# jby1993/SelfReconCode

Hardware: AMD Instinct MI355X
Metric: train.py-equivalent iterations/sec (540x540, 2048 rays/frame x 3 frames per GPU; coarse stage at Adam lr 0.0001) (higher is better)
Workload: dtype f32

## Files before the change

include/selfrecon_hip.h:

```cpp
#ifndef SELFRECON_HIP_H_
#define SELFRECON_HIP_H_
#include <stdint.h>

#ifdef __cplusplus
extern "C" {
#endif

#define SR_OK 0
#define SR_EINVAL (-1)
#define SR_ELAUNCH (-2)
#define SR_ENOSPC (-3)

int sr_abi_version(void);
const char* sr_build_arch(void);
const char* sr_build_digest(void);

int sr_minv3x3_fwd_f32(const float* ms, float* invs, uint8_t* checks, int64_t n, void* stream);
int sr_minv3x3_fwd_f64(const double* ms, double* invs, uint8_t* checks, int64_t n, void* stream);
int sr_minv3x3_bwd_f32(const float* grads, const float* invs, float* outs, int64_t n, void* stream);
int sr_minv3x3_bwd_f64(const double* grads, const double* invs, double* outs, int64_t n, void* stream);

typedef struct {
  int64_t size[5];
  int64_t stride[5];
} sr_tensor5;

int sr_gridsample3d_fwd_f32(const float* input, sr_tensor5 in_d, const float* grid, sr_tensor5 grid_d,
                            float* output, sr_tensor5 out_d, void* stream);
int sr_gridsample3d_fwd_f64(const double* input, sr_tensor5 in_d, const double* grid, sr_tensor5 grid_d,
                            double* output, sr_tensor5 out_d, void* stream);
int sr_gridsample3d_bwd_f32(const float* input, sr_tensor5 in_d, const float* grid, sr_tensor5 grid_d,
                            const float* grad_output, sr_tensor5 gout_d,
                            float* grad_input , sr_tensor5 gin_d, float* grad_grid, void* stream);
int sr_gridsample3d_bwd_f64(const double* input, sr_tensor5 in_d, const double* grid, sr_tensor5 grid_d,
                            const double* grad_output, sr_tensor5 gout_d,
                            double* grad_input , sr_tensor5 gin_d, double* grad_grid, void* stream);
int sr_gridsample3d_fwd_f16(const void* input, sr_tensor5 in_d, const void* grid, sr_tensor5 grid_d, void* output, sr_tensor5 out_d,
                            void* stream);
int sr_gridsample3d_bwd_f16(const void* input, sr_tensor5 in_d, const void* grid, sr_tensor5 grid_d, const void* grad_output,
                            sr_tensor5 gout_d, void* grad_input , sr_tensor5 gin_d, void* grad_grid, void* stream);
int sr_gridsample3d_dbwd_f16(const void* gO_input , sr_tensor5 goi_d, const void* gO_grid, sr_tensor5 gog_d,
                             const void* input, sr_tensor5 in_d, const void* grid, sr_tensor5 grid_d, const void* grad_output,
                             sr_tensor5 gout_d, void* grad_input , sr_tensor5 gin_d, void* grad_grid,
                             void* grad_grad_output, void* stream);
int sr_gridsample3d_dbwd_f32(const float* gO_input , sr_tensor5 goi_d, const float* gO_grid, sr_tensor5 gog_d,
                             const float* input, sr_tensor5 in_d, const float* grid, sr_tensor5 grid_d,
                             const float* grad_output, sr_tensor5 gout_d,
                             float* grad_input , sr_tensor5 gin_d, float* grad_grid, float* grad_grad_output,
                             void* stream);
int sr_gridsample3d_dbwd_f64(const double* gO_input , sr_tensor5 goi_d, const double* gO_grid, sr_tensor5 gog_d,
                             const double* input, sr_tensor5 in_d, const double* grid, sr_tensor5 grid_d,
                             const double* grad_output, sr_tensor5 gout_d,
                             double* grad_input , sr_tensor5 gin_d, double* grad_grid, double* grad_grad_output,
                             void* stream);


#define SR_ACT_NONE 0
#define SR_ACT_SOFTPLUS100 1
#define SR_ACT_RELU 2
#define SR_EPI_FWD 0
#define SR_EPI_BWD 1
typedef struct {
  const float* A; int64_t lda;
  const float* B; int64_t ldb;
  float* C; int64_t ldc;
  int32_t M, N, K;
  const float* bias;
  int32_t group, act, mode;
  float out_scale;
  const float* aux; int64_t ldaux;
  int32_t naux_fwd;
  int32_t nact_bwd;
  float aux_scale;
} sr_gemm_args;
int sr_mlp_gemm_nt(const sr_gemm_args* host_args, void* stream);
int sr_mlp_gemm_nt_tile(int32_t M, int32_t ncols, int32_t* bm_out, int32_t* bn_out);

#define SR_CHAIN_MAX_LAYERS 10
typedef struct {
  int32_t nlayers;
  int32_t nprob[SR_CHAIN_MAX_LAYERS];
  sr_gemm_args g[SR_CHAIN_MAX_LAYERS][2];
  const int32_t* m_dev; int32_t m_mul;
  int32_t m_cap;
} sr_chain_args;
int sr_mlp_chain(const sr_chain_args* host_args, void* stream);

typedef struct {
  const float* Z; int64_t ldz;
  const float* A; int64_t lda;
  float* dW; int64_t lddw;
  float* partial;
  int32_t R, N, K, splits, accumulate;
  float* db; float* db_partial; int32_t group;
} sr_gemm_tn_args;
int64_t sr_mlp_gemm_tn_workspace_floats(int32_t R, int32_t N, int64_t lddw, int32_t* host_splits_out);
int sr_mlp_gemm_tn(const sr_gemm_tn_args* host_args, void* stream);
#define SR_TN_GROUP_MAX 12
typedef struct {
  int32_t n;
  sr_gemm_tn_args p[SR_TN_GROUP_MAX];
} sr_gemm_tn_group_args;
int sr_mlp_gemm_tn_group(const sr_gemm_tn_group_args* host_args, void* stream);

int sr_pe_embed(const float* x, int64_t P, int32_t L, const float* band_weights, const float* extra, int64_t ldextra,
                int32_t E, const int64_t* extra_index , int32_t group, float* out, int64_t ldo, void* stream);
int sr_pe_embed_bwd(const float* x, int64_t P, int32_t L, const float* band_weights, int32_t group, const float* gA0,
                    int64_t ldg, float* xbar, void* stream);

typedef struct {
  const float* p; const float* tp; int64_t P;
  const float* A; const float* trans; int32_t nframes;
  const int64_t* batch_inds; int64_t points_per_frame;
  const float* vol; int32_t D, H, W;
  float bmin[3], bmax[3];
  float* y;
  float* jac;
} sr_lbs_args;
int sr_lbs_fwd(const sr_lbs_args* host_args, void* stream);
int64_t sr_lbs_bwd_workspace_floats(int64_t P, int32_t nframes);
int sr_lbs_bwd(const sr_lbs_args* host_args, const float* ybar, float* pbar, float* Abar, float* transbar, float* partials, void* stream);
int sr_lbs_jac_bwd(const sr_lbs_args* host_args, const float* ybar, const float* Jbar, float* pbar, float* Abar, float* transbar, float* partials,
                   void* stream);

int sr_lbs_chain_fwd(const float* poses, int32_t B, const float* host_Js, const int32_t* host_parents, const float* host_init_pose,
                     float* G, float* A, void* stream);
int sr_lbs_chain_bwd(const float* poses, int32_t B, const float* host_Js, const int32_t* host_parents, const float* host_init_pose,
                     const float* Abar, const float* Gbar, float* posebar, void* stream);

typedef struct {
  int64_t M; int32_t group;
  const float* sdf4; int64_t ld_sdf;
  const float* off4; int64_t ld_off;
  const float* y; const float* jlbs;
  const float* rays; const float* cam;
  const float* p; float* p_out;
  uint8_t* converged;
  float dthreshold, athreshold, w1, w2;
} sr_newton_args;
int sr_newton_update(const sr_newton_args* host_args, void* stream);

typedef struct {
  int64_t M;
  const float* sdf; int64_t ld_sdf;
  const float* y; const float* jlbs;
  const float* rays; const float* cam;
  uint8_t* converged;
  float* t_out; int64_t ld_t; float* s_out;
  const float* grad_f; const float* grad_off;
  const float* p; float* p_out;
  float dthreshold, athreshold, w1, w2;
} sr_newton2_args;
int sr_newton_prepare(const sr_newton2_args* host_args, void* stream);
int sr_newton_apply(const sr_newton2_args* host_args, void* stream);

typedef struct {
  int32_t P, times;
  const float* p0; const float* rays; const int64_t* batch_inds;
  const float* cam;
  int32_t L_sdf; const float* w_sdf; int32_t L_def; const float* w_def;
  const float* conds; int64_t ld_conds; int32_t E;
  const float* A; const float* trans; int32_t nframes;
  const float* vol; int32_t D, H, W; float bmin[3], bmax[3];
  float dthreshold, athreshold, w1, w2;
  int32_t* live;
  float* x[2]; float* v[2]; int32_t* frame[2]; int32_t* orig[2];
  float* unit;
  float* a0; int64_t ld_a0; float* a0d; int64_t ld_a0d;
  const float* sdf_out; int64_t ld_sdf; const float* def_out; int64_t ld_def;
  uint8_t* conv; float* t; float* s;
  const float* a0bar; int64_t ld_a0bar; const float* skipbar; int64_t ld_skipbar; int32_t n_skip;
  const float* a0dbar; int64_t ld_a0dbar;
  float* p_out; uint8_t* conv_out;
} sr_refine_args;
int sr_refine_init(const sr_refine_args* host_args, void* stream);
int sr_refine_embed(const sr_refine_args* host_args, int32_t phase, void* stream);
int sr_refine_mid(const sr_refine_args* host_args, int32_t phase, int32_t mode, void* stream);
int sr_refine_finish(const sr_refine_args* host_args, int32_t phase, void* stream);


int64_t sr_mc_workspace_bytes(int32_t nx, int32_t ny, int32_t nz);
int sr_mc_count(const float* sdf, int32_t nx, int32_t ny, int32_t nz, float iso, void* workspace, uint32_t* counts_dev, void* stream);
int sr_mc_emit(const float* sdf, int32_t nx, int32_t ny, int32_t nz, float iso, const void* workspace, float xstep, float ystep,
               float zstep, float xmin, float ymin, float zmin, float* verts, int64_t* faces, void* stream);

int sr_svd3x3(const float* A, int64_t n, float* U, float* S, float* V, void* stream);

int sr_rows_pad(const float* a, int64_t lda, int32_t na, const float* b, int64_t ldb, int32_t nb, int64_t rows, int32_t group, float* dst, int64_t ldd,
                int32_t width, void* stream);
int64_t sr_rows_frame_sum_workspace_floats(int64_t P, int32_t E, int32_t n);
int sr_rows_frame_sum(const float* X, int64_t ldx, int64_t P, int32_t E, const int64_t* index, int32_t n, float* partial, float* out, void* stream);

#define SR_PACK_MAX_LAYERS 16
typedef struct { const float* v; const float* g; float* W; float* WT; float* norms; int32_t N, K; int64_t ldw, ldwt; } sr_pack_layer;
typedef struct { int32_t nlayers; sr_pack_layer layer[SR_PACK_MAX_LAYERS]; } sr_pack_table;
typedef struct { const float* dW; int64_t lddw; const float* v; const float* g; const float* norms; float* gv; float* gg;
                 const float* db; float* gb;
                 int32_t N, K, accumulate, pad_; } sr_unpack_layer;
typedef struct { int32_t nlayers; sr_unpack_layer layer[SR_PACK_MAX_LAYERS]; } sr_unpack_table;
int sr_pack_weights(const sr_pack_table* host_table, void* stream);
int sr_unpack_grads(const sr_unpack_table* host_table, void* stream);

#define SR_ADAM_MAX_TENSORS 64
typedef struct { float* p; const float* g; float* m; float* v; int64_t numel; float lr, bias1, inv_sqrt_bias2, pad_; } sr_adam_tensor;
typedef struct { int32_t ntensors; float beta1, beta2, eps;
                 float one_minus_beta1, one_minus_beta2;
                 int32_t pad_[2]; sr_adam_tensor tensor[SR_ADAM_MAX_TENSORS]; } sr_adam_table;
int sr_adam_step(const sr_adam_table* host_table, void* stream);

int sr_stream_stamp(uint64_t* out, void* stream);
int sr_stream_flag_set(uint32_t* flag, uint32_t value, void* stream);
int sr_stream_flag_wait(const uint32_t* flag, uint32_t value, uint32_t* timed_out, int32_t timeout_ms, void* stream);

int sr_interp2x3d_fwd_f32(const float* in, int64_t BC, int32_t d, int32_t h, int32_t w, float balance, float* out, uint8_t* is_boundary, void* stream);
int sr_interp2x3d_fwd_f64(const double* in, int64_t BC, int32_t d, int32_t h, int32_t w, float balance, double* out, uint8_t* is_boundary, void* stream);
int sr_interp2x3d_bwd_f32(const float* grad_out, int64_t BC, int32_t d, int32_t h, int32_t w, float* grad_in, void* stream);
int sr_interp2x3d_bwd_f64(const double* grad_out, int64_t BC, int32_t d, int32_t h, int32_t w, double* grad_in, void* stream);
int sr_seg3d_candidates(const uint8_t* is_boundary, const uint8_t* done, int32_t D, int32_t H, int32_t W, int64_t* out_index, uint64_t* count_dev,
                        void* stream);

int64_t sr_points_silhouette_workspace_bytes(int64_t nimg, int64_t pts_per_img, int32_t H, int32_t W, float radius);
int sr_points_silhouette_fwd(const float* xy_ndc, const float* z, int64_t nimg, int64_t pts_per_img, int32_t H, int32_t W, float radius,
                             int32_t K, float* mask, void* workspace, void* stream);
int sr_points_silhouette_bwd(const float* xy_ndc, const float* z, int64_t nimg, int64_t pts_per_img, int32_t H, int32_t W, float radius,
                             const void* workspace, const float* gmask, float* gxy, void* stream);
int sr_rasterize_meshes(const float* xy_ndc, const float* z, const int64_t* faces, int64_t nimg, int64_t V, int64_t F, int32_t H, int32_t W,
                        void* zbuf_u64, int64_t* pix_to_face, float* bary, float* zout, void* stream);

int sr_vertex_adjacency(const int64_t* faces, int64_t V, int64_t F, int64_t* offsets, int32_t* cursor, int32_t* nbr, void* stream);
int sr_vertex_normals(const float* verts, int64_t N, int64_t V, const int64_t* offsets, const int32_t* nbr, float* normals, void* stream);
int sr_shade_phong(const float* verts, const float* normals, const int64_t* faces, int64_t N, int64_t V, int64_t F, int32_t H, int32_t W,
                   const int64_t* pix_to_face, const float* bary, const float* cam_pos, const float* light_loc, const float* host_phong,
                   float* rgba, void* stream);

#define SR_STEP_MAX_FRAMES 8
typedef struct { const float* R; const float* T; const float* f; const float* c; float W, H, one_minus_inv_w, one_minus_inv_h; } sr_camera;
int sr_step_reduce_blocks(int64_t rows);
int sr_step_param_blocks(int64_t rows);
int sr_cam_project_ndc_fwd(const float* ps, int64_t n, const sr_camera* cam, float* xy, float* z, void* stream);
int sr_cam_project_ndc_bwd(const float* ps, int64_t n, const sr_camera* cam, const float* gxy, const float* gz, float* gps, float* partial,
                           float* gparams, void* stream);
int sr_cam_view_rays_fwd(const float* pixels, int64_t n, const sr_camera* cam, float* rays, void* stream);
int sr_cam_view_rays_bwd(const float* pixels, int64_t n, const sr_camera* cam, const float* grays, float* partial, float* gparams, void* stream);

int sr_cardinal_rays_fwd(const float* J, const float* v, int64_t n, float* out, uint8_t* ok, void* stream);
int sr_cardinal_rays_bwd(const float* J, const float* v, int64_t n, const float* gout, float* gJ, float* gv, void* stream);
int sr_deformed_normals(const float* J, const float* onx, int64_t n, float* out, void* stream);

#define SR_STEP_LOSS_SLOTS (1 + 2 * SR_STEP_MAX_FRAMES)
typedef struct { const int64_t* b; const int64_t* r; const int64_t* c; int64_t P; int32_t N, H, W; } sr_ray_pixels;
int sr_color_loss_fwd(const sr_ray_pixels* px, const float* colors, const float* gt, float* partial, float* out, void* stream);
int sr_color_loss_bwd(const sr_ray_pixels* px, const float* colors, const float* gt, const float* saved, const float* gloss, float* gcolors,
                      void* stream);
int sr_normal_loss_fwd(const sr_ray_pixels* px, const float* nx_raw, const float* J, const float* gt_normals, const float* R, const float* rays,
                       int weighted, float* partial, float* out, void* stream);
int sr_normal_loss_bwd(const sr_ray_pixels* px, const float* nx_raw, const float* J, const float* gt_normals, const float* R, const float* rays,
                       int weighted, const float* saved, const float* gloss, float* gnx_raw, float* gJ, void* stream);
int sr_eikonal_loss_fwd(const float* g, int64_t n, float* partial, float* out, void* stream);
int sr_eikonal_loss_bwd(const float* g, int64_t n, const float* gloss, float* gg, void* stream);
int sr_def_regu_loss_fwd(const float* S, int64_t n, float c, float* partial, float* out, void* stream);
int sr_def_regu_loss_bwd(const float* U, const float* S, const float* V, int64_t n, float c, const float* gloss, float* gJ, void* stream);
int sr_svd3x3_bwd(const float* U, const float* V, const float* gS, int64_t n, float* gJ, void* stream);
int sr_mask_iou_loss_fwd(const float* masks, const float* gt, int N, int64_t hw, float* partial, float* out, void* stream);
int sr_mask_iou_loss_bwd(const float* masks, const float* gt, int N, int64_t hw, const float* saved, const float* gloss, float* gmasks, void* stream);

int sr_implicit_solve(const float* grad_f, const float* J, const float* v, const float* grad_l, int64_t n, float* cot_f, float* rhs_tail, float* temp,
                      uint8_t* ok, void* stream);

int sr_uv_rasterize(const float* vt, const int64_t* ft, int64_t Vt, int64_t F, int32_t R, int32_t* face, float* bary, void* stream);
int sr_face_visibility(const int64_t* pix_to_face, const int64_t* faces, int64_t N, int64_t V, int64_t F, const float* xy_pix, const uint8_t* mask,
                       int32_t H, int32_t W, uint8_t* visible, void* stream);
int sr_view_alpha(const float* verts, const float* normals, const float* cam_pos, int64_t N, int64_t V, float* alpha, void* stream);
int sr_texture_accumulate(int64_t T, const int32_t* tface, const float* tbary, const int64_t* faces, int64_t F, int64_t V, int32_t N,
                          const uint8_t* visible, const float* alpha, const float* xy_pix, const float* images, int32_t H, int32_t W,
                          const int32_t* fids, int32_t agg_num, float cosv0, float* slot_cos, float* slot_rgb, int32_t* slot_view, int32_t* count,
                          float* min_cos, int32_t* min_idx, void* stream);
int sr_texture_resolve(int64_t T, const int32_t* texel, int32_t agg_num, float cosv0, int32_t check_num, const float* slot_cos,
                       const float* slot_rgb, const int32_t* slot_view, int32_t* count, uint8_t* mask_final, int32_t* view_id, float* tex_median,
                       void* stream);
int64_t sr_texture_fill_workspace_bytes(int32_t R);
int sr_texture_fill(const float* tex_median, const uint8_t* mask_final, const uint8_t* tex_mask, int32_t R, int32_t dilate, float* texture,
                    void* workspace, void* stream);

#define SR_QUADRIC_CLAMPED 1
#define SR_QUADRIC_NO_PLANES 2
int sr_meshprep_cell_faces(const int64_t* faces, int64_t F, const int64_t* vertex_map, int64_t V, int64_t C, int64_t* slot, void* stream);
int sr_meshprep_cell_quadric(const float* verts, int64_t V, const int64_t* faces, int64_t F, const int64_t* face_slots, const int64_t* face_offsets,
                             const int64_t* order, const int64_t* offsets, const int64_t* cells, int64_t C, const float* lo, float cell, int64_t nx,
                             int64_t ny, double reg, float* out, int32_t* flags, float* shift, void* stream);
int sr_meshprep_face_flips(const float* verts, int64_t V, const int64_t* faces, int64_t F, const float* new_verts, int64_t Vn,
                           const int64_t* new_faces, const int64_t* source, int64_t Fn, int64_t* counts, void* stream);
int sr_meshprep_bounds(const float* verts, int64_t V, int32_t* box, void* stream);
int sr_meshprep_cell_keys(const float* verts, int64_t V, const float* lo, float cell, int64_t nx, int64_t ny, int64_t nz, int64_t* key, void* stream);
int sr_meshprep_cell_mean(const float* verts, int64_t V, const int64_t* order, const int64_t* offsets, int64_t C, float* out, void* stream);
int sr_meshprep_face_keys(const int64_t* faces, int64_t F, const int64_t* vertex_map, int64_t V, int64_t Vn, int64_t* out_faces, int64_t* key_hi,
                          int64_t* key_lo, void* stream);
int sr_meshprep_face_first(const int64_t* key_hi, const int64_t* key_lo, const int64_t* perm, int64_t F, uint8_t* keep, void* stream);
int sr_chart_classify(const float* verts, int64_t V, const int64_t* faces, int64_t F, int32_t* cls, void* stream);
int sr_chart_edge_keys(const int64_t* faces, int64_t F, int64_t V, const int32_t* cls, int64_t* key, void* stream);
int sr_chart_hook(const int64_t* sorted_key, const int64_t* perm, int64_t n, const int32_t* parent, int32_t* next, int64_t F, int32_t* changed,
                  void* stream);
int sr_chart_jump(const int32_t* parent, int64_t F, int32_t* next, int32_t* changed, void* stream);
int sr_chart_bbox(const float* verts, int64_t V, const int64_t* faces, int64_t F, const int32_t* cls, const int64_t* chart, int64_t C, int32_t* box,
                  float* bbox_min, float* extent, void* stream);
int sr_chart_uv(const float* verts, int64_t V, const int64_t* faces, int64_t F, const int32_t* cls, const int64_t* chart, int64_t C,
                const float* bbox_min, const int64_t* origin, double scale, int32_t padding, int32_t R, float* vt, void* stream);
int sr_uv_overlap_count(const float* vt, const int64_t* ft, int64_t Vt, int64_t F, int32_t R, double eps, int32_t* count, int64_t* total,
                        void* stream);

int sr_collapse_vertex_quadrics(const float* verts, int64_t V, const int64_t* faces, int64_t F, const int64_t* slots, const int64_t* offsets,
                                double* quadrics, void* stream);
int sr_collapse_edge_keys(const int64_t* faces, int64_t F, int64_t V, int64_t* key, void* stream);
int sr_collapse_edge_heads(const int64_t* unique_key, const int64_t* offsets, int64_t E, const int64_t* perm, const int64_t* faces, int64_t F, int64_t V,
                           int64_t* edges, int32_t* count, int64_t* opposite, int32_t* locked, int64_t* directed, void* stream);
int sr_collapse_candidates(const float* verts, int64_t V, const int64_t* faces, int64_t F, const double* quadrics, const int64_t* slots,
                           const int64_t* offsets, const int64_t* neighbours, const int64_t* neighbour_offsets, const int64_t* edges,
                           const int32_t* count, const int64_t* opposite, const int32_t* locked, int64_t E, double reg, double flip_cos,
                           float* positions, int64_t* key, void* stream);
int sr_collapse_min1(const int64_t* edges, const int64_t* key, int64_t E, int64_t V, int64_t* m1, void* stream);
int sr_collapse_min2(const int64_t* edges, int64_t E, int64_t V, const int64_t* m1, int64_t* m2, void* stream);
int sr_collapse_select(const int64_t* edges, const int64_t* key, int64_t E, int64_t V, const int64_t* m2, uint8_t* selected, int64_t* record,
                       void* stream);
int sr_collapse_apply_vertices(const int64_t* edges, const float* positions, const uint8_t* selected, int64_t E, float* verts, int64_t V,
                               double* quadrics, int64_t* target, void* stream);
int sr_collapse_apply_faces(const int64_t* faces, int64_t F, const int64_t* target, int64_t V, int64_t* out_faces, uint8_t* keep, void* stream);
int sr_collapse_map_jump(const int64_t* parent, int64_t V, int64_t* next, int32_t* changed, void* stream);

int sr_texture_mips(const void* texture, int32_t is_u8, const uint8_t* valid, int32_t R, float* mips, void* stream);
int sr_texture_face_lod(const float* xy_pix, const int64_t* faces, const float* vt, const int64_t* ft, int64_t N, int64_t V, int64_t F,
                        int64_t Vt, int32_t R, float bias, int32_t L, float* lod, void* stream);
int sr_shade_textured(const int64_t* pix_to_face, const float* bary, int64_t N, int64_t F, int32_t H, int32_t W, const int64_t* ft,
                      const float* vt, int64_t Vt, const float* mips, int32_t R, int32_t L, const float* lod, const float* host_background,
                      const float* host_hole, const float* bg_image, float* rgba, float* coverage, void* stream);

#define SR_LBSW_MAX_K 32
int sr_lbsw_knn_blend(const float* verts, const float* vert_ws, int64_t nv, int32_t nj, int32_t k, int32_t W, int32_t H, int32_t D,
                      const float* bmin, const float* bmax, int32_t align_corners, float* field, void* stream);
int sr_lbsw_smooth(const float* src, float* dst, int32_t nj, int32_t W, int32_t H, int32_t D, void* stream);

#define SR_SMPL_BATCH_TILE 8
int sr_smpl_shape(const float* v_template, const float* shapedirs, const float* beta, int32_t B, int32_t nbeta, int64_t nv, float* v_shaped,
                  void* stream);
int64_t sr_smpl_regress_workspace_floats(int32_t B, int64_t nv, int32_t nk);
int sr_smpl_regress(const float* x, const float* reg, int32_t B, int64_t nv, int32_t nk, float* partial, float* out, void* stream);
int sr_smpl_pose(const float* theta, float* Rs, const float* J, const int32_t* host_parents, int32_t B, float* feature, float* J_transformed,
                 float* A, void* stream);
int sr_smpl_skin(const float* rest, int64_t rest_batch_stride, const float* posedirs, const float* feature, const float* weights, const float* A,
                 int32_t B, int64_t nv, float* verts, void* stream);

int sr_smpl_regress_bwd(const float* g_out, const float* reg, int32_t B, int64_t nv, int32_t nk, int32_t accumulate, float* g_x, void* stream);
int64_t sr_smpl_shape_bwd_workspace_floats(int32_t B, int32_t nbeta, int64_t nv);
int sr_smpl_shape_bwd(const float* shapedirs, const float* g_vshaped, int32_t B, int32_t nbeta, int64_t nv, float* partial, float* g_beta,
                      void* stream);
int64_t sr_smpl_skin_bwd_workspace_floats(int32_t B, int64_t nv);
int sr_smpl_skin_bwd(const float* rest, int64_t rest_batch_stride, const float* posedirs, const float* feature, const float* weights,
                     const float* A, const float* gV, int32_t B, int64_t nv, float* partial, float* g_rest, float* gA, float* g_feature,
                     void* stream);
int sr_smpl_pose_bwd(const float* theta, const float* Rs, const float* J, const float* A, const int32_t* host_parents, int32_t B,
                     const float* gA, const float* gJ_transformed, const float* g_feature, const float* gRs, float* g_theta, float* gRs_out,
                     float* gJ, void* stream);

int sr_keypoint_energy(const float* joints, const float* trans, const float* kp, const float* joint_weights, const float* host_camera,
                       float sigma, int32_t T, int32_t K, float* energy, float* g_joints, float* g_trans, int32_t* behind, void* stream);

#define SR_EDT_EMPTY 1073741824
int sr_edt(const uint8_t* mask, int32_t F, int32_t H, int32_t W, int32_t* d2, void* stream);
int sr_contour_flags(const uint8_t* mask, int32_t F, int32_t H, int32_t W, uint8_t* flags, void* stream);
int sr_silhouette_energy(const float* points, const int32_t* d2, const int32_t* samples, const int32_t* counts, const float* host_camera,
                         float sigma, float margin, int32_t F, int32_t V, int32_t S, int32_t H, int32_t W, float* xy, uint8_t* valid,
                         float* vres, int32_t* match, float* sres, float* e_in, float* e_cov, int32_t* outside, float* g_points, void* stream);

#define SR_MESHREG_LAP 1
#define SR_MESHREG_EDGE 2
#define SR_MESHREG_NORMAL 4
int64_t sr_meshreg_workspace_bytes(int64_t V, int64_t P);
int sr_meshreg_fwd(const float* verts, int64_t V, const int32_t* nbr_row, const int32_t* nbr, int64_t E, const int32_t* pairs, int64_t P,
                   int32_t terms, float target_length, float* lap_q, float* edge_g, float* pair_g, void* workspace, float* out, void* stream);
int sr_meshreg_bwd(int64_t V, const int32_t* nbr_row, const int32_t* nbr, int64_t E, const int32_t* pair_row, const int32_t* pair_ent, int64_t P,
                   const float* lap_q, const float* edge_g, const float* pair_g, const float* g_lap, const float* g_edge, const float* g_nc,
                   float* grad, void* stream);

#define SR_FRAMES_MAX_BATCH 16
#define SR_FRAMES_MAX_PIXELS 1073741824
struct sr_frame_ids_s {
  int32_t id[SR_FRAMES_MAX_BATCH];
};
typedef struct sr_frame_ids_s sr_frame_ids;
int sr_frames_fetch(const uint8_t* img_u8, const uint8_t* normal_u8, const uint8_t* mask_u8, int64_t pitch3, int64_t pitch1, int32_t F, int32_t H,
                    int32_t W, const sr_frame_ids* ids_by_value, const int64_t* ids_device, int32_t N, float* out_img, float* out_normal,
                    float* out_mask, void* stream);

#define SR_LOG_MAX_SLOTS 32
#define SR_LOG_EMPTY 0
#define SR_LOG_F32 1
#define SR_LOG_I64 2
#define SR_LOG_IMM 3
struct sr_log_slots_s {
  const void* src[SR_LOG_MAX_SLOTS];
  float imm[SR_LOG_MAX_SLOTS];
  uint8_t kind[SR_LOG_MAX_SLOTS];
};
typedef struct sr_log_slots_s sr_log_slots;
int sr_log_row(const sr_log_slots* slots_by_value, int32_t n, float* ring, int32_t ring_rows, int32_t ld, int64_t row, void* stream);

#define SR_JPEG_BLOCK_BYTES 208
int sr_jpeg_transform(const uint8_t* rgb, int32_t B, int32_t H, int32_t W, const uint16_t* qtab, int16_t* coef, void* stream);
int sr_jpeg_entropy(const int16_t* coef, int32_t B, int32_t H, int32_t W, const uint32_t* huff, uint32_t* bits, int64_t bits_dwords,
                    uint8_t* rowbuf, int64_t rowbuf_bytes, uint32_t* row_len, void* stream);
int sr_jpeg_gather(const uint8_t* rowbuf, const uint32_t* row_len, int32_t B, int32_t H, int32_t W, int64_t* row_start, uint8_t* out,
                   int64_t out_bytes, int64_t* offsets, void* stream);

int sr_surfdist_face_cells(const float* tri, int64_t F, const float* lo, float cell, int32_t nx, int32_t ny, int32_t nz, int64_t* count, void* stream);
int sr_surfdist_emit_pairs(const float* tri, int64_t F, const float* lo, float cell, int32_t nx, int32_t ny, int32_t nz, const int64_t* offset,
                           int64_t pairs, int64_t* key, int32_t* pair_face, void* stream);
int sr_surfdist_query(const float* points, int64_t P, const float* tri, int64_t F, const float* lo, float cell, int32_t nx, int32_t ny, int32_t nz,
                      const int64_t* cell_start, const int32_t* cell_faces, int64_t pairs, float* dist, int64_t* face, float* closest, void* stream);
int sr_surfdist_brute(const float* points, int64_t P, const float* tri, int64_t F, float* dist, int64_t* face, float* closest, void* stream);
int sr_mesh_sample(const float* tri, const double* cum_area, int64_t F, int64_t n, int64_t seed, float* points, int64_t* face, float* normals,
                   void* stream);

#define SR_ICP_MAX_BLOCKS 1024
#define SR_ICP_COLS 40
#define SR_ICP_HISTORY 6
#define SR_ICP_STATE 16
#define SR_ICP_DONE 12
int sr_icp_accumulate(const float* points, int64_t S, const float* tri, int64_t F, const float* lo, float cell, int32_t nx, int32_t ny, int32_t nz,
                      const int64_t* cell_start, const int32_t* cell_faces, int64_t pairs, const double* state, double ox, double oy, double oz,
                      double rho, float max_dist, int32_t measure, double* partial, int32_t blocks, void* stream);
int sr_icp_solve(const double* partial, int32_t blocks, double ox, double oy, double oz, double rho, int32_t scale, double tol, int32_t it,
                 int32_t iters, double* state, double* history, void* stream);
int sr_icp_score(const float* points, int64_t S, const double* table, int32_t N, const float* tri, int64_t F, const float* lo, float cell,
                 int32_t nx, int32_t ny, int32_t nz, const int64_t* cell_start, const int32_t* cell_faces, int64_t pairs, const float* trunc,
                 double* score, void* stream);

#ifdef __cplusplus
}
#endif
#endif
```

selfreconcode_amd/csrc/mlp_gemm.hip:

```cpp
#include "sr_common.h"
#include <stdlib.h>
#include <type_traits>

typedef float f32x16 __attribute__((ext_vector_type(16)));
typedef float f32x4 __attribute__((ext_vector_type(4)));
typedef int i32x4 __attribute__((ext_vector_type(4)));

__device__ __forceinline__ __amdgpu_buffer_rsrc_t sr_make_rsrc(const void* base, int64_t bytes) {
  return __builtin_amdgcn_make_buffer_rsrc(const_cast<void*>(base), 0, (int)(bytes < 0xFFFFFFFFll ? bytes : 0xFFFFFFFFll), 0x00020000);
}
__device__ __forceinline__ f32x4 sr_buffer_load16(__amdgpu_buffer_rsrc_t rsrc, uint32_t lane_off, uint32_t scalar_off) {
  return __builtin_bit_cast(f32x4, __builtin_amdgcn_raw_buffer_load_b128(rsrc, (int)lane_off, (int)scalar_off, 0));
}

namespace {

constexpr int BK = 32;
constexpr int LDSP = BK + 4;

__device__ __forceinline__ float fast_exp(float x) { return __builtin_amdgcn_exp2f(x * 1.4426950408889634f); }
__device__ __forceinline__ float fast_log(float x) { return __builtin_amdgcn_logf(x) * 0.6931471805599453f; }
__device__ __forceinline__ float softplus100(float z) {
  const float t = z * 100.0f;
  const float e = fast_exp(fminf(t, 20.0f));
  const float l = e < 1e-3f ? e * (1.0f - e * (0.5f - e * 0.33333334f)) : fast_log(1.0f + e);
  return t > 20.0f ? z : l * 0.01f;
}
__device__ __forceinline__ float dsoftplus100(float z) {
  const float t = z * 100.0f;
  const float e = fast_exp(fminf(t, 20.0f));
  return t > 20.0f ? 1.0f : e * __builtin_amdgcn_rcpf(e + 1.0f);
}
__device__ __forceinline__ void softplus100_from_stored(float x, float& d, float& c2) {
  const float em = fast_exp(-x);
  d = x < 1e-3f ? x * (1.0f - x * (0.5f - x * 0.16666667f)) : 1.0f - em;
  c2 = 100.0f * em;
}

template <int WM, int WN, int TM, int TN>
struct Cfg {
  static constexpr int kWaves = WM * WN;
  static constexpr int kThreads = kWaves * 64;
  static constexpr int BM = WM * TM * 32;
  static constexpr int BN = WN * TN * 32;
  static constexpr int kALoads = BM * (BK / 4) / kThreads;
  static constexpr int kBLoads = (BN * (BK / 4) + kThreads - 1) / kThreads;
  static constexpr int kOperandFloats = 2 * (BM + BN) * LDSP;
  static constexpr int kStageFloats = kWaves * TM * 32 * (TN * 32 + 4);
  static constexpr int kLdsFloats = kOperandFloats > kStageFloats ? kOperandFloats : kStageFloats;
};

template <int ROWS, int NLOADS, int THREADS>
struct TileLoader {
  const float* p[NLOADS];
  __amdgpu_buffer_rsrc_t rsrc;
  uint32_t off[NLOADS];
  int kq4;
  int K, kmax;
  __device__ __forceinline__ TileLoader(const float* __restrict__ P, int64_t ld, int R, int K_, int r0) : K(K_) {
    kq4 = (threadIdx.x & 7) * 4;
    kmax = ((K_ + 3) & ~3) - 4;
    const int rb = r0 < R ? r0 : R - 1;
    rsrc = sr_make_rsrc(P + (int64_t)rb * ld, (int64_t)(R - rb) * ld * 4);
#pragma unroll
    for (int j = 0; j < NLOADS; ++j) {
      int row = (threadIdx.x + j * THREADS) >> 3;
      if (row >= ROWS) row = ROWS - 1;
      int gr = r0 + row;
      if (gr >= R) gr = R - 1;
      p[j] = P + (int64_t)gr * ld;
      off[j] = (uint32_t)(((int64_t)(gr - rb) * ld + kq4) * 4);
    }
  }
  __device__ __forceinline__ void load(int k0, f32x4 (&reg)[NLOADS]) const {
    const int gk = k0 + kq4;
    const int gkc = gk < kmax ? gk : kmax;
#pragma unroll
    for (int j = 0; j < NLOADS; ++j) reg[j] = *reinterpret_cast<const f32x4*>(p[j] + gkc);
  }
  __device__ __forceinline__ void load_full(int k0, int klast, f32x4 (&reg)[NLOADS]) const {
    const uint32_t kc = (uint32_t)(k0 < klast ? k0 : klast) * 4u;
#pragma unroll
    for (int j = 0; j < NLOADS; ++j) reg[j] = sr_buffer_load16(rsrc, off[j], kc);
  }
  template <bool KTAIL = true>
  __device__ __forceinline__ void store(float* __restrict__ lds, int k0, const f32x4 (&reg)[NLOADS]) const {
    const int nvalid = K - (k0 + kq4);
#pragma unroll
    for (int j = 0; j < NLOADS; ++j) {
      const int idx = threadIdx.x + j * THREADS;
      const int row = idx >> 3;
      f32x4 v = reg[j];
      if (KTAIL) { v.x = nvalid > 0 ? v.x : 0.f; v.y = nvalid > 1 ? v.y : 0.f; v.z = nvalid > 2 ? v.z : 0.f; v.w = nvalid > 3 ? v.w : 0.f; }
      if (ROWS * 8 % THREADS == 0 || row < ROWS) *reinterpret_cast<f32x4*>(lds + row * LDSP + kq4) = v;
    }
  }
};

template <int WM, int WN, int TM, int TN, int G>
__device__ __forceinline__ void epilogue(const sr_gemm_args& g, f32x16 (&acc)[TM][TN], int m0, int n0, int wm, int wn,
                                         int li, int kh, float* __restrict__ stage) {
  constexpr int SP = TN * 32 + 4;
  const int ncols = g.N + g.naux_fwd;
  const float inv_aux_scale = 1.0f / g.aux_scale;
#pragma unroll
  for (int a = 0; a < TM; ++a) {
#pragma unroll
    for (int b = 0; b < TN; ++b) {
      const int col = n0 + (wn * TN + b) * 32 + li;
      if (col >= ncols) continue;
      const float bias = (g.bias && col < g.N) ? g.bias[col] : 0.f;
#pragma unroll
      for (int q = 0; q < 4; ++q) {
        const int r0 = m0 + (wm * TM + a) * 32 + 8 * q + 4 * kh;
        if (r0 >= g.M) continue;
        float v[4] = {acc[a][b][4 * q], acc[a][b][4 * q + 1], acc[a][b][4 * q + 2], acc[a][b][4 * q + 3]};
        float o[4];
        if (g.mode == SR_EPI_FWD) {
          if (col >= g.N) {
#pragma unroll
            for (int j = 0; j < 4; ++j) o[j] = (r0 + j < g.M) ? g.aux[(int64_t)(r0 + j) * g.ldaux + (col - g.N)] * g.out_scale : 0.f;
          } else {
#pragma unroll
            for (int s = 0; s < 4; s += G) {
              const float z = v[s] + bias;
              float d;
              if (g.act == SR_ACT_SOFTPLUS100) { o[s] = softplus100(z) * g.out_scale; d = (G > 1) ? dsoftplus100(z) : 0.f; }
              else if (g.act == SR_ACT_RELU) { o[s] = fmaxf(z, 0.f) * g.out_scale; d = z > 0.f ? 1.f : 0.f; }
              else { o[s] = z * g.out_scale; d = 1.f; }
#pragma unroll
              for (int tI = 1; tI < G; ++tI) o[s + tI] = d * v[s + tI] * g.out_scale;
            }
          }
        } else {
          if (col >= g.nact_bwd) {
#pragma unroll
            for (int j = 0; j < 4; ++j) o[j] = v[j] * g.out_scale;
          } else {
            float sv[4];
#pragma unroll
            for (int j = 0; j < 4; ++j) sv[j] = (r0 + j < g.M) ? g.aux[(int64_t)(r0 + j) * g.ldaux + col] : 0.f;
#pragma unroll
            for (int s = 0; s < 4; s += G) {
              float d, c2;
              if (g.act == SR_ACT_SOFTPLUS100) {
                softplus100_from_stored(100.0f * (sv[s] * inv_aux_scale), d, c2);
              } else if (g.act == SR_ACT_RELU) { d = sv[s] > 0.f ? 1.f : 0.f; c2 = 0.f; }
              else { d = 1.f; c2 = 0.f; }
              float cross = 0.f;
#pragma unroll
              for (int tI = 1; tI < G; ++tI) {
                cross += sv[s + tI] * v[s + tI];
                o[s + tI] = d * g.aux_scale * v[s + tI];
              }
              o[s] = d * g.aux_scale * v[s] + c2 * cross;
            }
          }
        }
        float* sp = stage + (a * 32 + 8 * q + 4 * kh) * SP + b * 32 + li;
#pragma unroll
        for (int j = 0; j < 4; ++j) sp[j * SP] = o[j];
      }
    }
  }
  __syncthreads();
  constexpr int QPR = TN * 8;
  constexpr int RPI = 64 / QPR;
  const int lane = kh * 32 + li;
  const int qc = lane % QPR, ro = lane / QPR;
  const int col0 = n0 + wn * TN * 32 + qc * 4;
#pragma unroll
  for (int i = 0; i < TM * 32 / RPI; ++i) {
    const int lr = i * RPI + ro;
    const int row = m0 + wm * TM * 32 + lr;
    if (row >= g.M || col0 >= ncols) continue;
    const f32x4 v = *reinterpret_cast<const f32x4*>(stage + lr * SP + qc * 4);
    float* dst = g.C + (int64_t)row * g.ldc + col0;
    if (col0 + 3 < ncols) {
      *reinterpret_cast<f32x4*>(dst) = v;
    } else {
      dst[0] = v.x;
      if (col0 + 1 < ncols) dst[1] = v.y;
      if (col0 + 2 < ncols) dst[2] = v.z;
    }
  }
}

template <int WM, int WN, int TM, int TN, int G, int MODE, int ACT>
__device__ __forceinline__ void epilogue_interior(const sr_gemm_args& g, f32x16 (&acc)[TM][TN], int m0, int n0, int wm, int wn, int li,
                                                  int kh, float* __restrict__ stage) {
  constexpr int SP = TN * 32 + 4;
  const float os = g.out_scale, as = g.aux_scale, inv_as = 1.0f / g.aux_scale;
#pragma unroll
  for (int a = 0; a < TM; ++a) {
#pragma unroll
    for (int b = 0; b < TN; ++b) {
      const int col = n0 + (wn * TN + b) * 32 + li;
      const float bias = (MODE == SR_EPI_FWD && g.bias) ? g.bias[col] : 0.f;
#pragma unroll
      for (int q = 0; q < 4; ++q) {
        const int r0 = m0 + (wm * TM + a) * 32 + 8 * q + 4 * kh;
        const float v[4] = {acc[a][b][4 * q], acc[a][b][4 * q + 1], acc[a][b][4 * q + 2], acc[a][b][4 * q + 3]};
        float o[4];
        if constexpr (MODE == SR_EPI_FWD) {
#pragma unroll
          for (int s = 0; s < 4; s += G) {
            const float z = v[s] + bias;
            float d = 1.f;
            if constexpr (ACT == SR_ACT_SOFTPLUS100) { o[s] = softplus100(z) * os; if (G > 1) d = dsoftplus100(z); }
            else if constexpr (ACT == SR_ACT_RELU) { o[s] = fmaxf(z, 0.f) * os; d = z > 0.f ? 1.f : 0.f; }
            else { o[s] = z * os; }
#pragma unroll
            for (int tI = 1; tI < G; ++tI) o[s + tI] = d * v[s + tI] * os;
          }
        } else {
          float sv[4];
          if constexpr (ACT != SR_ACT_NONE || G > 1) {
            const float* ap = g.aux + (int64_t)r0 * g.ldaux + col;
#pragma unroll
            for (int j = 0; j < 4; ++j) sv[j] = ap[(int64_t)j * g.ldaux];
          }
#pragma unroll
          for (int s = 0; s < 4; s += G) {
            float d = 1.f, c2 = 0.f;
            if constexpr (ACT == SR_ACT_SOFTPLUS100) softplus100_from_stored(100.0f * (sv[s] * inv_as), d, c2);
            else if constexpr (ACT == SR_ACT_RELU) d = sv[s] > 0.f ? 1.f : 0.f;
            float cross = 0.f;
#pragma unroll
            for (int tI = 1; tI < G; ++tI) {
              cross += sv[s + tI] * v[s + tI];
              o[s + tI] = d * as * v[s + tI];
            }
            o[s] = d * as * v[s] + c2 * cross;
          }
        }
        float* sp = stage + (a * 32 + 8 * q + 4 * kh) * SP + b * 32 + li;
#pragma unroll
        for (int j = 0; j < 4; ++j) sp[j * SP] = o[j];
      }
    }
  }
  __syncthreads();
  constexpr int QPR = TN * 8, RPI = 64 / QPR;
  const int lane = kh * 32 + li;
  const int qc = lane % QPR, ro = lane / QPR;
  float* dst = g.C + (int64_t)(m0 + wm * TM * 32 + ro) * g.ldc + n0 + wn * TN * 32 + qc * 4;
#pragma unroll
  for (int i = 0; i < TM * 32 / RPI; ++i)
    *reinterpret_cast<f32x4*>(dst + (int64_t)i * RPI * g.ldc) = *reinterpret_cast<const f32x4*>(stage + (i * RPI + ro) * SP + qc * 4);
}

template <int WM, int WN, int TM, int TN, int G, int MODE>
__device__ __forceinline__ void epilogue_interior_act(const sr_gemm_args& g, f32x16 (&acc)[TM][TN], int m0, int n0, int wm, int wn, int li,
                                                      int kh, float* __restrict__ stage) {
  if (g.act == SR_ACT_SOFTPLUS100) epilogue_interior<WM, WN, TM, TN, G, MODE, SR_ACT_SOFTPLUS100>(g, acc, m0, n0, wm, wn, li, kh, stage);
  else if (g.act == SR_ACT_RELU) epilogue_interior<WM, WN, TM, TN, G, MODE, SR_ACT_RELU>(g, acc, m0, n0, wm, wn, li, kh, stage);
  else epilogue_interior<WM, WN, TM, TN, G, MODE, SR_ACT_NONE>(g, acc, m0, n0, wm, wn, li, kh, stage);
}

struct NoProbe { __device__ __forceinline__ void operator()(int) const {} };
template <int WM, int WN, int TM, int TN, bool KTAIL = true, class Probe = NoProbe>
__device__ __forceinline__ void gemm_nt_tile(const sr_gemm_args& g, int wg, float* __restrict__ smem, Probe probe = Probe()) {
  using C_ = Cfg<WM, WN, TM, TN>;
  auto As = [&](int buf) -> float* { return smem + buf * (C_::BM * LDSP); };
  auto Bs = [&](int buf) -> float* { return smem + 2 * C_::BM * LDSP + buf * (C_::BN * LDSP); };

  const int tiles_n = (g.N + g.naux_fwd + C_::BN - 1) / C_::BN;
  const int tiles_m = (g.M + C_::BM - 1) / C_::BM;
  const int nwg = tiles_m * tiles_n;
  {
    const int q = nwg / 8, r = nwg % 8, xcd = wg % 8, loc = wg / 8;
    wg = (xcd < r ? xcd * (q + 1) : r * (q + 1) + (xcd - r) * q) + loc;
  }
  const int tn = wg % tiles_n, tm = wg / tiles_n;
  const int m0 = tm * C_::BM, n0 = tn * C_::BN;

  const int lane = threadIdx.x & 63, wave = threadIdx.x >> 6;
  const int wm = wave / WN, wn = wave % WN;
  const int li = lane & 31, kh = lane >> 5;

  f32x16 acc[TM][TN];
#pragma unroll
  for (int a = 0; a < TM; ++a)
#pragma unroll
    for (int b = 0; b < TN; ++b)
#pragma unroll
      for (int r = 0; r < 16; ++r) acc[a][b][r] = 0.f;

  const TileLoader<C_::BM, C_::kALoads, C_::kThreads> la(g.A, g.lda, g.M, g.K, m0);
  const TileLoader<C_::BN, C_::kBLoads, C_::kThreads> lb(g.B, g.ldb, g.N, g.K, n0);
  const int nk = (g.K + BK - 1) / BK;
  const int a_off = (wm * TM * 32 + li) * LDSP + kh * 4, b_off = (wn * TN * 32 + li) * LDSP + kh * 4;
  f32x4 fa0[2][TM], fb0[2][TN], fa1[2][TM], fb1[2][TN];
  auto read_frags = [&](const float* abuf, const float* bbuf, int kk0, f32x4 (&fa)[2][TM], f32x4 (&fb)[2][TN]) {
#pragma unroll
    for (int h = 0; h < 2; ++h) {
#pragma unroll
      for (int a = 0; a < TM; ++a) fa[h][a] = *reinterpret_cast<const f32x4*>(abuf + a_off + a * 32 * LDSP + (kk0 + h) * 8);
#pragma unroll
      for (int b = 0; b < TN; ++b) fb[h][b] = *reinterpret_cast<const f32x4*>(bbuf + b_off + b * 32 * LDSP + (kk0 + h) * 8);
    }
  };
  auto mfma_kk = [&](const f32x4 (&fa)[TM], const f32x4 (&fb)[TN]) {
#pragma unroll
    for (int e = 0; e < 4; ++e)
#pragma unroll
      for (int a = 0; a < TM; ++a)
#pragma unroll
        for (int b = 0; b < TN; ++b) acc[a][b] = __builtin_amdgcn_mfma_f32_32x32x2f32(fa[a][e], fb[b][e], acc[a][b], 0, 0, 0);
  };
  constexpr int kMem = C_::kALoads + C_::kBLoads;

  f32x4 ra0[C_::kALoads], rb0[C_::kBLoads], ra1[C_::kALoads], rb1[C_::kBLoads];
  const int klast = (nk - 1) * BK;
  auto load_tile = [&](int k0, f32x4 (&ar)[C_::kALoads], f32x4 (&br)[C_::kBLoads]) {
    if constexpr (KTAIL) { la.load(k0, ar); lb.load(k0, br); }
    else { la.load_full(k0, klast, ar); lb.load_full(k0, klast, br); }
  };
  load_tile(0, ra0, rb0);
  load_tile(BK, ra1, rb1);
  la.template store<KTAIL>(As(0), 0, ra0); lb.template store<KTAIL>(Bs(0), 0, rb0);
  __syncthreads();
  read_frags(As(0), Bs(0), 0, fa0, fb0);
  probe(0);
  auto step = [&](int t, f32x4 (&ain)[C_::kALoads], f32x4 (&bin)[C_::kBLoads], const f32x4 (&aout)[C_::kALoads],
                  const f32x4 (&bout)[C_::kBLoads]) {
    const int cur = t & 1;
    load_tile((t + 2) * BK, ain, bin);
    la.template store<KTAIL>(As(cur ^ 1), (t + 1) * BK, aout); lb.template store<KTAIL>(Bs(cur ^ 1), (t + 1) * BK, bout);
    read_frags(As(cur), Bs(cur), 2, fa1, fb1);
    mfma_kk(fa0[0], fb0[0]);
    mfma_kk(fa0[1], fb0[1]);
#pragma unroll
    for (int i = 0; i < kMem; ++i) {
      __builtin_amdgcn_sched_group_barrier(0x020, 1, 0);
      __builtin_amdgcn_sched_group_barrier(0x008, 1, 0);
    }
#pragma unroll
    for (int i = 0; i < kMem; ++i) {
      __builtin_amdgcn_sched_group_barrier(0x200, 1, 0);
      __builtin_amdgcn_sched_group_barrier(0x008, 1, 0);
    }
#pragma unroll
    for (int i = 0; i < 2 * (TM + TN); ++i) {
      __builtin_amdgcn_sched_group_barrier(0x100, 1, 0);
      __builtin_amdgcn_sched_group_barrier(0x008, 1, 0);
    }
    __builtin_amdgcn_sched_barrier(0);
    __syncthreads();
    read_frags(As(cur ^ 1), Bs(cur ^ 1), 0, fa0, fb0);
    __builtin_amdgcn_sched_barrier(0);
    mfma_kk(fa1[0], fb1[0]);
    mfma_kk(fa1[1], fb1[1]);
    __builtin_amdgcn_sched_barrier(0);
  };
  for (int t = 0; t < nk; t += 2) {
    step(t, ra0, rb0, ra1, rb1);
    if (t + 1 < nk) step(t + 1, ra1, rb1, ra0, rb0);
  }
  __syncthreads();
  probe(1);

  float* stage = smem + wave * (TM * 32 * (TN * 32 + 4));
  const bool interior = m0 + C_::BM <= g.M && n0 + C_::BN <= (g.mode == SR_EPI_FWD ? g.N : (g.nact_bwd < g.N ? g.nact_bwd : g.N));
  if (interior) {
    if (g.mode == SR_EPI_FWD) {
      switch (g.group) {
        case 1: epilogue_interior_act<WM, WN, TM, TN, 1, SR_EPI_FWD>(g, acc, m0, n0, wm, wn, li, kh, stage); break;
        case 2: epilogue_interior_act<WM, WN, TM, TN, 2, SR_EPI_FWD>(g, acc, m0, n0, wm, wn, li, kh, stage); break;
        default: epilogue_interior_act<WM, WN, TM, TN, 4, SR_EPI_FWD>(g, acc, m0, n0, wm, wn, li, kh, stage); break;
      }
    } else {
      switch (g.group) {
        case 1: epilogue_interior_act<WM, WN, TM, TN, 1, SR_EPI_BWD>(g, acc, m0, n0, wm, wn, li, kh, stage); break;
        case 2: epilogue_interior_act<WM, WN, TM, TN, 2, SR_EPI_BWD>(g, acc, m0, n0, wm, wn, li, kh, stage); break;
        default: epilogue_interior_act<WM, WN, TM, TN, 4, SR_EPI_BWD>(g, acc, m0, n0, wm, wn, li, kh, stage); break;
      }
    }
  } else {
    switch (g.group) {
      case 1: epilogue<WM, WN, TM, TN, 1>(g, acc, m0, n0, wm, wn, li, kh, stage); break;
      case 2: epilogue<WM, WN, TM, TN, 2>(g, acc, m0, n0, wm, wn, li, kh, stage); break;
      default: epilogue<WM, WN, TM, TN, 4>(g, acc, m0, n0, wm, wn, li, kh, stage); break;
    }
  }
  probe(2);
}

template <int WM, int WN, int TM, int TN, bool KTAIL>
__global__ __launch_bounds__(WM * WN * 64) __attribute__((amdgpu_waves_per_eu(2))) void gemm_nt_kernel(sr_gemm_args g) {
  extern __shared__ __attribute__((aligned(16))) float smem[];
  gemm_nt_tile<WM, WN, TM, TN, KTAIL>(g, blockIdx.x, smem);
}


using ChainCfg = Cfg<2, 2, 1, 1>;

constexpr int TBR = 32;
template <int ZW, int XW>
struct TnCfg {
  static constexpr int ZLD = ZW + 4, XLD = XW + 4;
  static constexpr int kZ = TBR * ZLD, kX = TBR * XLD;
  static constexpr int kLdsFloats = 2 * (kZ + kX);
  static constexpr int TLZ = TBR * (ZW / 4) / 256, TLX = TBR * (XW / 4) / 256;
  static constexpr int WN = XW / 64;
};

template <int ZW, int XW>
__device__ __forceinline__ void gemm_tn_body(const sr_gemm_tn_args& g, int rows_per_split, int bid, int nblocks, float* __restrict__ tn_smem) {
  using C = TnCfg<ZW, XW>;
  auto Zs = [&](int buf) -> float* { return tn_smem + buf * C::kZ; };
  auto Xs = [&](int buf) -> float* { return tn_smem + 2 * C::kZ + buf * C::kX; };
  const int tiles_k = (g.K + XW - 1) / XW;
  const int tiles_n = (g.N + ZW - 1) / ZW;
  int vb = bid;
  if ((nblocks & 7) == 0) vb = (bid & 7) * (nblocks >> 3) + (bid >> 3);
  const int tile = vb % (tiles_k * tiles_n), split = vb / (tiles_k * tiles_n);
  const int n0 = (tile / tiles_k) * ZW, k0 = (tile % tiles_k) * XW;
  const int r_begin = split * rows_per_split;
  const int r_end = min(g.R, r_begin + rows_per_split);
  const int lane = threadIdx.x & 63, wave = threadIdx.x >> 6;
  const int wm = wave / C::WN, wn = wave % C::WN, li = lane & 31, kh = lane >> 5;

  f32x16 acc[2][2];
#pragma unroll
  for (int a = 0; a < 2; ++a)
#pragma unroll
    for (int b = 0; b < 2; ++b)
#pragma unroll
      for (int r = 0; r < 16; ++r) acc[a][b][r] = 0.f;

  constexpr int TLZ = C::TLZ, TLX = C::TLX;
  constexpr int ZT = ZW / 4, XT = XW / 4;
  const int cqz = (threadIdx.x % ZT) * 4, lrz = threadIdx.x / ZT;
  const int cqx = (threadIdx.x % XT) * 4, lrx = threadIdx.x / XT;
  const int zmax = ((g.N + 3) & ~3) - 4, xmax = ((g.K + 3) & ~3) - 4;
  const float* zcol = g.Z + (n0 + cqz < zmax ? n0 + cqz : zmax);
  const float* xcol = g.A + (k0 + cqx < xmax ? k0 + cqx : xmax);
  f32x4 rz[TLZ], rx[TLX];
  const __amdgpu_buffer_rsrc_t zrsrc = sr_make_rsrc(g.Z + (int64_t)r_begin * g.ldz, (int64_t)(g.R - r_begin) * g.ldz * 4);
  const __amdgpu_buffer_rsrc_t xrsrc = sr_make_rsrc(g.A + (int64_t)r_begin * g.lda, (int64_t)(g.R - r_begin) * g.lda * 4);
  uint32_t zbyte[TLZ], xbyte[TLX];
#pragma unroll
  for (int j = 0; j < TLZ; ++j) zbyte[j] = (uint32_t)(((int64_t)(lrz + j * (256 / ZT)) * g.ldz + (zcol - g.Z)) * 4);
#pragma unroll
  for (int j = 0; j < TLX; ++j) xbyte[j] = (uint32_t)(((int64_t)(lrx + j * (256 / XT)) * g.lda + (xcol - g.A)) * 4);
  const int last_full = r_end - TBR;
  auto load = [&](int r0, auto tail) {
    if constexpr (decltype(tail)::value) {
#pragma unroll
      for (int j = 0; j < TLZ; ++j) {
        int gr = r0 + lrz + j * (256 / ZT);
        gr = gr < r_end ? gr : r_end - 1;
        rz[j] = *reinterpret_cast<const f32x4*>(zcol + (int64_t)gr * g.ldz);
      }
#pragma unroll
      for (int j = 0; j < TLX; ++j) {
        int gr = r0 + lrx + j * (256 / XT);
        gr = gr < r_end ? gr : r_end - 1;
        rx[j] = *reinterpret_cast<const f32x4*>(xcol + (int64_t)gr * g.lda);
      }
    } else {
      const int rc = r0 < last_full ? r0 : last_full;
      const uint32_t zo = (uint32_t)((int64_t)(rc - r_begin) * g.ldz * 4), xo = (uint32_t)((int64_t)(rc - r_begin) * g.lda * 4);
#pragma unroll
      for (int j = 0; j < TLZ; ++j) rz[j] = sr_buffer_load16(zrsrc, zbyte[j], zo);
#pragma unroll
      for (int j = 0; j < TLX; ++j) rx[j] = sr_buffer_load16(xrsrc, xbyte[j], xo);
    }
  };
  auto store = [&](int buf, int r0, auto tail) {
    float* zs = Zs(buf);
    float* xs = Xs(buf);
#pragma unroll
    for (int j = 0; j < TLZ; ++j) {
      const int row = lrz + j * (256 / ZT);
      f32x4 z = rz[j];
      if constexpr (decltype(tail)::value) {
        const bool ok = r0 + row < r_end;
        z.x = ok ? z.x : 0.f; z.y = ok ? z.y : 0.f; z.z = ok ? z.z : 0.f; z.w = ok ? z.w : 0.f;
      }
      *reinterpret_cast<f32x4*>(zs + row * C::ZLD + cqz) = z;
    }
#pragma unroll
    for (int j = 0; j < TLX; ++j) {
      const int row = lrx + j * (256 / XT);
      f32x4 x = rx[j];
      if constexpr (decltype(tail)::value) {
        const bool ok = r0 + row < r_end;
        x.x = ok ? x.x : 0.f; x.y = ok ? x.y : 0.f; x.z = ok ? x.z : 0.f; x.w = ok ? x.w : 0.f;
      }
      *reinterpret_cast<f32x4*>(xs + row * C::XLD + cqx) = x;
    }
  };

  constexpr int HS = TBR / 4;
  typedef float f32x2 __attribute__((ext_vector_type(2)));
  float z0a[HS], z1a[HS], x0a[HS], x1a[HS], z0b[HS], z1b[HS], x0b[HS], x1b[HS];
  const int zoff = kh * C::ZLD + wm * 64 + 2 * li, xoff = kh * C::XLD + wn * 64 + 2 * li;
  auto read_half = [&](int buf, int half, float (&z0)[HS], float (&z1)[HS], float (&x0)[HS], float (&x1)[HS]) {
    const float* zb = Zs(buf) + zoff + half * HS * 2 * C::ZLD;
    const float* xb = Xs(buf) + xoff + half * HS * 2 * C::XLD;
#pragma unroll
    for (int e = 0; e < HS; ++e) {
      const f32x2 z = *reinterpret_cast<const f32x2*>(zb + 2 * e * C::ZLD), x = *reinterpret_cast<const f32x2*>(xb + 2 * e * C::XLD);
      z0[e] = z.x; z1[e] = z.y; x0[e] = x.x; x1[e] = x.y;
    }
  };
  auto mfma_half = [&](const float (&z0)[HS], const float (&z1)[HS], const float (&x0)[HS], const float (&x1)[HS]) {
#pragma unroll
    for (int e = 0; e < HS; ++e) {
      acc[0][0] = __builtin_amdgcn_mfma_f32_32x32x2f32(z0[e], x0[e], acc[0][0], 0, 0, 0);
      acc[0][1] = __builtin_amdgcn_mfma_f32_32x32x2f32(z0[e], x1[e], acc[0][1], 0, 0, 0);
      acc[1][0] = __builtin_amdgcn_mfma_f32_32x32x2f32(z1[e], x0[e], acc[1][0], 0, 0, 0);
      acc[1][1] = __builtin_amdgcn_mfma_f32_32x32x2f32(z1[e], x1[e], acc[1][1], 0, 0, 0);
    }
  };

  const bool do_bias = g.db_partial != nullptr && k0 == 0;
  const float wodd = g.group == 4 ? 0.f : 1.f;
  float bsum0 = 0.f, bsum1 = 0.f;
  auto bias_half = [&](const float (&z0)[HS], const float (&z1)[HS]) {
#pragma unroll
    for (int e = 0; e < HS; ++e) {
      if (e & 1) { bsum0 += wodd * z0[e]; bsum1 += wodd * z1[e]; }
      else { bsum0 += z0[e]; bsum1 += z1[e]; }
    }
  };
  const int nsteps = (r_end - r_begin + TBR - 1) / TBR;
  auto run = [&](auto tail, auto bias) {
    load(r_begin, tail);
    store(0, r_begin, tail);
    load(r_begin + TBR, tail);
    __syncthreads();
    read_half(0, 0, z0a, z1a, x0a, x1a);
    for (int t = 0; t < nsteps; ++t) {
      const int cur = t & 1;
      store(cur ^ 1, r_begin + (t + 1) * TBR, tail);
      load(r_begin + (t + 2) * TBR, tail);
      read_half(cur, 1, z0b, z1b, x0b, x1b);
      mfma_half(z0a, z1a, x0a, x1a);
#pragma unroll
      for (int i = 0; i < TLZ + TLX; ++i) {
        __builtin_amdgcn_sched_group_barrier(0x200, 1, 0);
        __builtin_amdgcn_sched_group_barrier(0x008, 1, 0);
      }
#pragma unroll
      for (int i = 0; i < TLZ + TLX; ++i) {
        __builtin_amdgcn_sched_group_barrier(0x020, 1, 0);
        __builtin_amdgcn_sched_group_barrier(0x008, 1, 0);
      }
#pragma unroll
      for (int i = 0; i < HS; ++i) {
        __builtin_amdgcn_sched_group_barrier(0x100, 1, 0);
        __builtin_amdgcn_sched_group_barrier(0x008, 1, 0);
      }
      __builtin_amdgcn_sched_barrier(0);
      if constexpr (decltype(bias)::value) bias_half(z0a, z1a);
      __builtin_amdgcn_sched_barrier(0);
      __syncthreads();
      read_half(cur ^ 1, 0, z0a, z1a, x0a, x1a);
      __builtin_amdgcn_sched_barrier(0);
      mfma_half(z0b, z1b, x0b, x1b);
      if constexpr (decltype(bias)::value) bias_half(z0b, z1b);
      __builtin_amdgcn_sched_barrier(0);
    }
  };
  if (nsteps > 0) {
    const bool tail = ((r_end - r_begin) % TBR) != 0;
    if (tail) {
      if (do_bias) run(std::true_type{}, std::true_type{}); else run(std::true_type{}, std::false_type{});
    } else {
      if (do_bias) run(std::false_type{}, std::true_type{}); else run(std::false_type{}, std::false_type{});
    }
  }
  __syncthreads();
  if (do_bias) {
    float* red = Zs(0);
    if (wn == 0) {
      const bool use = kh == 0 || g.group == 1;
      red[kh * ZW + wm * 64 + 2 * li] = use ? bsum0 : 0.f;
      red[kh * ZW + wm * 64 + 2 * li + 1] = use ? bsum1 : 0.f;
    }
    __syncthreads();
    if (threadIdx.x < ZW && n0 + threadIdx.x < g.N) g.db_partial[(int64_t)split * g.N + n0 + threadIdx.x] = red[threadIdx.x] + red[threadIdx.x + ZW];
  }
  float* out = g.partial + (int64_t)split * g.N * g.lddw;
#pragma unroll
  for (int a = 0; a < 2; ++a)
#pragma unroll
    for (int b = 0; b < 2; ++b) {
      const int col = k0 + wn * 64 + 2 * li + b;
      if (col >= g.K) continue;
#pragma unroll
      for (int r = 0; r < 16; ++r) {
        const int row = n0 + wm * 64 + 2 * ((r & 3) + 8 * (r >> 2) + 4 * kh) + a;
        if (row < g.N) out[(int64_t)row * g.lddw + col] = acc[a][b][r];
      }
    }
}

template <int ZW, int XW>
__global__ __launch_bounds__(256) __attribute__((amdgpu_waves_per_eu(2))) void gemm_tn_kernel(sr_gemm_tn_args g, int rows_per_split) {
  extern __shared__ __attribute__((aligned(16))) float tn_smem[];
  gemm_tn_body<ZW, XW>(g, rows_per_split, blockIdx.x, gridDim.x, tn_smem);
}

struct TnGroup {
  int n;
  int first[SR_TN_GROUP_MAX + 1];
  int blocks[SR_TN_GROUP_MAX];
  int rows_per_split[SR_TN_GROUP_MAX];
  sr_gemm_tn_args p[SR_TN_GROUP_MAX];
};
__global__ __launch_bounds__(256) __attribute__((amdgpu_waves_per_eu(2))) void gemm_tn_group_kernel(TnGroup G) {
  extern __shared__ __attribute__((aligned(16))) float tn_smem[];
  int i = 0;
  while (i + 1 < G.n && (int)blockIdx.x >= G.first[i + 1]) ++i;
  const int bid = blockIdx.x - G.first[i];
  if (bid >= G.blocks[i]) return;
  gemm_tn_body<128, 128>(G.p[i], G.rows_per_split[i], bid, G.blocks[i], tn_smem);
}

static inline bool tn_narrow(int N, int64_t K) { return K <= 64 && N >= 256; }

__device__ __forceinline__ void slab_reduce_body(const float* __restrict__ partial, float* __restrict__ dW, int N,
                                                 int K, int64_t lddw, int splits, int accumulate,
                                                 const float* __restrict__ db_partial, float* __restrict__ db, int bid, int nblocks) {
  const int64_t total = (int64_t)N * lddw;
  const int64_t quads = total >> 2;
  const int64_t all = quads + (db ? N : 0);
  const f32x4* __restrict__ p4 = reinterpret_cast<const f32x4*>(partial);
  f32x4* __restrict__ d4 = reinterpret_cast<f32x4*>(dW);
  for (int64_t i = (int64_t)bid * blockDim.x + threadIdx.x; i < all; i += (int64_t)nblocks * blockDim.x) {
    if (i < quads) {
      const int col = (int)((i << 2) % lddw);
      f32x4 s = {0.f, 0.f, 0.f, 0.f};
      if (col < K) {
        const f32x4* src = p4 + i;
        int p = 0;
        for (; p + 8 <= splits; p += 8) {
          f32x4 v[8];
#pragma unroll
          for (int j = 0; j < 8; ++j) v[j] = src[(int64_t)(p + j) * quads];
#pragma unroll
          for (int j = 0; j < 8; ++j) s += v[j];
        }
        for (; p < splits; ++p) s += src[(int64_t)p * quads];
        if (col + 1 >= K) s.y = 0.f;
        if (col + 2 >= K) s.z = 0.f;
        if (col + 3 >= K) s.w = 0.f;
      }
      f32x4 o = {0.f, 0.f, 0.f, 0.f};
      if (accumulate) o = d4[i];
      d4[i] = o + s;
    } else {
      const int n = (int)(i - quads);
      float s = 0.f;
      for (int p = 0; p < splits; ++p) s += db_partial[(int64_t)p * N + n];
      db[n] = (accumulate ? db[n] : 0.f) + s;
    }
  }
}

__global__ __launch_bounds__(256) void slab_reduce_kernel(const float* __restrict__ partial, float* __restrict__ dW, int N,
                                                           int K, int64_t lddw, int splits, int accumulate,
                                                           const float* __restrict__ db_partial, float* __restrict__ db) {
  slab_reduce_body(partial, dW, N, K, lddw, splits, accumulate, db_partial, db, blockIdx.x, gridDim.x);
}

__global__ __launch_bounds__(256) void slab_reduce_group_kernel(TnGroup G) {
  int i = 0;
  while (i + 1 < G.n && (int)blockIdx.x >= G.first[i + 1]) ++i;
  const int bid = blockIdx.x - G.first[i];
  if (bid >= G.blocks[i]) return;
  const sr_gemm_tn_args& g = G.p[i];
  slab_reduce_body(g.partial, g.dW, g.N, g.K, g.lddw, g.R > 0 ? g.splits : 0, g.accumulate, g.db_partial, g.db, bid, G.blocks[i]);
}

}

static void nt_tile_choice(int M, int ncols, int* bm, int* bn) {
  auto cost = [&](int tm, int tn, double eff) {
    const int64_t wgs = sr_cdiv(M, tm) * sr_cdiv(ncols, tn);
    return (double)sr_cdiv(wgs, 256) * tm * tn / eff;
  };
  if (ncols <= 32) {
    const double c[3] = {cost(32, 32, 0.6), cost(64, 32, 0.8), cost(256, 32, 1.0)};
    *bn = 32;
    if (c[0] < c[1] && c[0] < c[2]) *bm = 32;
    else if (c[1] < c[2]) *bm = 64;
    else *bm = 256;
  } else {
    const double c[3] = {cost(64, 64, 0.92), cost(64, 128, 0.94), cost(128, 128, 1.0)};
    int pick = 1;
    for (int i = 1; i < 3; ++i) if (c[i] < c[pick - 1]) pick = i + 1;
    *bm = pick == 3 ? 128 : 64;
    *bn = pick == 1 ? 64 : 128;
  }
}

extern "C" {
int sr_mlp_gemm_nt(const sr_gemm_args* a, void* stream) {
  if (!a || a->M < 0 || a->N <= 0 || a->K <= 0) return SR_EINVAL;
  if (a->M == 0) return SR_OK;
  if (!a->A || !a->B || !a->C) return SR_EINVAL;
  if (a->group != 1 && a->group != 2 && a->group != 4) return SR_EINVAL;
  if ((a->lda & 3) || (a->ldb & 3) || (a->ldc & 3) || ((uintptr_t)a->A & 15) || ((uintptr_t)a->B & 15) || ((uintptr_t)a->C & 15)) return SR_EINVAL;
  if (a->mode != SR_EPI_FWD && a->mode != SR_EPI_BWD) return SR_EINVAL;
  if ((a->naux_fwd > 0 || a->mode == SR_EPI_BWD) && a->act != SR_ACT_NONE && !a->aux && a->mode == SR_EPI_BWD) return SR_EINVAL;
  if (a->mode == SR_EPI_FWD && a->naux_fwd > 0 && !a->aux) return SR_EINVAL;
  if (a->M == 0) return SR_OK;
  if (a->M % a->group) return SR_EINVAL;
  const int ncols = a->N + (a->mode == SR_EPI_FWD ? a->naux_fwd : 0);
  sr_gemm_args g = *a;
  if (g.mode != SR_EPI_FWD) g.naux_fwd = 0;
#define SR_NT_LAUNCH(WM, WN, TM, TN)                                                                                        \
  do {                                                                                                                      \
    using C_ = Cfg<WM, WN, TM, TN>;                                                                                         \
    const int nwg = (int)(sr_cdiv(g.M, C_::BM) * sr_cdiv(ncols, C_::BN));                                                   \
    if (g.K % BK)                                                                                                           \
      hipLaunchKernelGGL((gemm_nt_kernel<WM, WN, TM, TN, true>), dim3(nwg), dim3(C_::kThreads), C_::kLdsFloats * sizeof(float), \
                         (hipStream_t)stream, g);                                                                           \
    else                                                                                                                    \
      hipLaunchKernelGGL((gemm_nt_kernel<WM, WN, TM, TN, false>), dim3(nwg), dim3(C_::kThreads), C_::kLdsFloats * sizeof(float), \
                         (hipStream_t)stream, g);                                                                           \
  } while (0)
  int bm = 0, bn = 0;
  nt_tile_choice(g.M, ncols, &bm, &bn);
  switch (bm * 1024 + bn) {
    case 32 * 1024 + 32: SR_NT_LAUNCH(1, 1, 1, 1); break;
    case 64 * 1024 + 32: SR_NT_LAUNCH(2, 1, 1, 1); break;
    case 256 * 1024 + 32: SR_NT_LAUNCH(4, 1, 2, 1); break;
    case 64 * 1024 + 64: SR_NT_LAUNCH(2, 2, 1, 1); break;
    case 64 * 1024 + 128: SR_NT_LAUNCH(2, 2, 1, 2); break;
    default: SR_NT_LAUNCH(2, 2, 2, 2); break;
  }
#undef SR_NT_LAUNCH
  return sr_launch_status();
}

int sr_mlp_gemm_nt_tile(int32_t M, int32_t ncols, int32_t* bm, int32_t* bn) {
  if (M <= 0 || ncols <= 0 || !bm || !bn) return SR_EINVAL;
  nt_tile_choice(M, ncols, bm, bn);
  return SR_OK;
}

__global__ __launch_bounds__(ChainCfg::kThreads) __attribute__((amdgpu_waves_per_eu(2))) void mlp_layer_pair_kernel(sr_gemm_args g0, sr_gemm_args g1, int nprob,
                                                                                                                     const int32_t* __restrict__ m_dev, int m_mul) {
  extern __shared__ __attribute__((aligned(16))) float smem[];
  const int M = *m_dev * m_mul;
  if (M <= 0) return;
  const int rows = (M + ChainCfg::BM - 1) / ChainCfg::BM;
  const int t0 = rows * ((g0.N + (g0.mode == SR_EPI_FWD ? g0.naux_fwd : 0) + ChainCfg::BN - 1) / ChainCfg::BN);
  const int t1 = nprob > 1 ? rows * ((g1.N + (g1.mode == SR_EPI_FWD ? g1.naux_fwd : 0) + ChainCfg::BN - 1) / ChainCfg::BN) : 0;
  const int t = blockIdx.x;
  if (t >= t0 + t1) return;
  if (t < t0) { g0.M = M; if (g0.K % BK) gemm_nt_tile<2, 2, 1, 1, true>(g0, t, smem); else gemm_nt_tile<2, 2, 1, 1, false>(g0, t, smem); }
  else { g1.M = M; if (g1.K % BK) gemm_nt_tile<2, 2, 1, 1, true>(g1, t - t0, smem); else gemm_nt_tile<2, 2, 1, 1, false>(g1, t - t0, smem); }
}

int sr_mlp_chain(const sr_chain_args* a, void* stream) {
  if (!a || a->nlayers < 1 || a->nlayers > SR_CHAIN_MAX_LAYERS || !a->m_dev || a->m_mul < 1 || a->m_cap <= 0) return SR_EINVAL;
  for (int l = 0; l < a->nlayers; ++l) {
    if (a->nprob[l] < 1 || a->nprob[l] > 2) return SR_EINVAL;
    for (int p = 0; p < a->nprob[l]; ++p) {
      const sr_gemm_args& g = a->g[l][p];
      if (!g.A || !g.B || !g.C || g.N <= 0 || g.K <= 0 || g.group != a->m_mul) return SR_EINVAL;
      if ((g.lda & 3) || (g.ldb & 3) || (g.ldc & 3) || ((uintptr_t)g.A & 15) || ((uintptr_t)g.B & 15) || ((uintptr_t)g.C & 15)) return SR_EINVAL;
      if (g.mode != SR_EPI_FWD && g.mode != SR_EPI_BWD) return SR_EINVAL;
      if (g.mode == SR_EPI_BWD && g.naux_fwd != 0) return SR_EINVAL;
      if ((g.mode == SR_EPI_BWD && g.act != SR_ACT_NONE && !g.aux) || (g.mode == SR_EPI_FWD && g.naux_fwd > 0 && !g.aux)) return SR_EINVAL;
    }
  }
  const int64_t rows = sr_cdiv((int64_t)a->m_cap * a->m_mul, ChainCfg::BM);
  for (int l = 0; l < a->nlayers; ++l) {
    int64_t tiles = 0;
    for (int p = 0; p < a->nprob[l]; ++p) {
      const sr_gemm_args& g = a->g[l][p];
      tiles += rows * sr_cdiv(g.N + (g.mode == SR_EPI_FWD ? g.naux_fwd : 0), ChainCfg::BN);
    }
    hipLaunchKernelGGL(mlp_layer_pair_kernel, dim3((unsigned)tiles), dim3(ChainCfg::kThreads), ChainCfg::kLdsFloats * sizeof(float), (hipStream_t)stream,
                       a->g[l][0], a->g[l][a->nprob[l] > 1 ? 1 : 0], a->nprob[l], a->m_dev, a->m_mul);
  }
  return sr_launch_status();
}

int64_t sr_mlp_gemm_tn_workspace_floats(int32_t R, int32_t N, int64_t lddw, int32_t* splits_out) {
  const int tiles = tn_narrow(N, lddw) ? (int)sr_cdiv(N, 256) : (int)(sr_cdiv(N, 128) * sr_cdiv(lddw, 128));
  const int target = 512;
  int splits = (int)sr_cdiv(target, tiles);
  const int max_splits = (int)sr_cdiv(R, 384);
  if (splits > max_splits) splits = max_splits;
  if (splits < 1) splits = 1;
  if (splits_out) *splits_out = splits;
  return (int64_t)splits * N * lddw;
}

int sr_mlp_gemm_tn(const sr_gemm_tn_args* a, void* stream) {
  if (!a || !a->dW || !a->partial || a->R < 0 || a->N <= 0 || a->K <= 0 || a->splits < 1) return SR_EINVAL;
  if (a->R > 0 && (!a->Z || !a->A)) return SR_EINVAL;
  if ((a->ldz & 3) || (a->lda & 3) || ((uintptr_t)a->Z & 15) || ((uintptr_t)a->A & 15) || a->lddw < a->K) return SR_EINVAL;
  if ((a->lddw & 3) || ((uintptr_t)a->dW & 15) || ((uintptr_t)a->partial & 15)) return SR_EINVAL;
  if ((a->db != nullptr) != (a->db_partial != nullptr) || (a->db && a->group < 1)) return SR_EINVAL;
  const bool narrow = tn_narrow(a->N, a->lddw);
  const int tiles = narrow ? (int)sr_cdiv(a->N, 256) : (int)(sr_cdiv(a->N, 128) * sr_cdiv(a->K, 128));
  int rows_per_split = (int)sr_cdiv(a->R, a->splits);
  rows_per_split = (int)(sr_cdiv(rows_per_split, TBR) * TBR);
  if (a->R > 0) {
    using Narrow = TnCfg<256, 64>;
    using Square = TnCfg<128, 128>;
    if (narrow)
      hipLaunchKernelGGL((gemm_tn_kernel<256, 64>), dim3(tiles * a->splits), dim3(256), Narrow::kLdsFloats * sizeof(float), (hipStream_t)stream, *a,
                         rows_per_split);
    else
      hipLaunchKernelGGL((gemm_tn_kernel<128, 128>), dim3(tiles * a->splits), dim3(256), Square::kLdsFloats * sizeof(float), (hipStream_t)stream, *a,
                         rows_per_split);
  }
  const int64_t total = (int64_t)a->N * a->lddw / 4 + (a->db ? a->N : 0);
  sr_launch_stream(slab_reduce_kernel, total, 256, stream, a->partial, a->dW, a->N, a->K, a->lddw, a->R > 0 ? a->splits : 0, a->accumulate, a->db_partial,
                   a->db);
  return sr_launch_status();
}

static int tn_check(const sr_gemm_tn_args* a) {
  if (!a || !a->dW || !a->partial || a->R < 0 || a->N <= 0 || a->K <= 0 || a->splits < 1) return SR_EINVAL;
  if (a->R > 0 && (!a->Z || !a->A)) return SR_EINVAL;
  if ((a->ldz & 3) || (a->lda & 3) || ((uintptr_t)a->Z & 15) || ((uintptr_t)a->A & 15) || a->lddw < a->K) return SR_EINVAL;
  if ((a->lddw & 3) || ((uintptr_t)a->dW & 15) || ((uintptr_t)a->partial & 15)) return SR_EINVAL;
  if ((a->db != nullptr) != (a->db_partial != nullptr) || (a->db && a->group < 1)) return SR_EINVAL;
  return SR_OK;
}

int sr_mlp_gemm_tn_group(const sr_gemm_tn_group_args* a, void* stream) {
  if (!a || a->n < 1 || a->n > SR_TN_GROUP_MAX) return SR_EINVAL;
  TnGroup G, Rd;
  G.n = Rd.n = a->n;
  int nb = 0, nr = 0;
  bool any_rows = false;
  for (int i = 0; i < a->n; ++i) {
    const sr_gemm_tn_args& p = a->p[i];
    const int rc = tn_check(&p);
    if (rc != SR_OK) return rc;
    if (tn_narrow(p.N, p.lddw)) return SR_EINVAL;
    const int tiles = (int)(sr_cdiv(p.N, 128) * sr_cdiv(p.K, 128));
    int rows_per_split = (int)sr_cdiv(p.R, p.splits);
    rows_per_split = (int)(sr_cdiv(rows_per_split, TBR) * TBR);
    G.p[i] = Rd.p[i] = p;
    G.rows_per_split[i] = Rd.rows_per_split[i] = rows_per_split;
    G.first[i] = nb; G.blocks[i] = p.R > 0 ? tiles * p.splits : 0;
    nb += (int)(sr_cdiv(G.blocks[i], 8) * 8);
    const int64_t total = (int64_t)p.N * p.lddw / 4 + (p.db ? p.N : 0);
    Rd.first[i] = nr; Rd.blocks[i] = sr_stream_grid(total, 256);
    nr += Rd.blocks[i];
    any_rows = any_rows || p.R > 0;
  }
  G.first[a->n] = nb; Rd.first[a->n] = nr;
  using Square = TnCfg<128, 128>;
  if (any_rows && nb > 0)
    hipLaunchKernelGGL(gemm_tn_group_kernel, dim3(nb), dim3(256), Square::kLdsFloats * sizeof(float), (hipStream_t)stream, G);
  hipLaunchKernelGGL(slab_reduce_group_kernel, dim3(nr), dim3(256), 0, (hipStream_t)stream, Rd);
  return sr_launch_status();
}
}

namespace {
__global__ __launch_bounds__(256) void pe_embed_kernel(const float* __restrict__ x, int64_t P, int L, const float* __restrict__ w,
                                                        const float* __restrict__ extra, int64_t ldextra, int E,
                                                        const int64_t* __restrict__ extra_index, int group,
                                                        float* __restrict__ out, int64_t ldo) {
  const int width = 3 + 6 * L + E;
  const int64_t total = P * ldo;
  for (int64_t i = (int64_t)blockIdx.x * blockDim.x + threadIdx.x; i < total; i += (int64_t)gridDim.x * blockDim.x) {
    const int64_t p = i / ldo;
    const int c = (int)(i % ldo);
    float v = 0.f, t3[3] = {0.f, 0.f, 0.f};
    if (c < 3) {
      v = x[p * 3 + c];
      t3[c] = 1.f;
    } else if (c < 3 + 6 * L) {
      const int k = (c - 3) / 6, r = (c - 3) % 6, comp = r % 3;
      const float f = (float)(1 << k);
      const float a = x[p * 3 + comp] * f;
      const float wk = w[2 * k + (r >= 3)];
      if (r < 3) { v = wk * sinf(a); t3[comp] = wk * f * cosf(a); }
      else { v = wk * cosf(a); t3[comp] = -wk * f * sinf(a); }
    } else if (c < width) {
      const int64_t src = extra_index ? extra_index[p] : p;
      v = extra[src * ldextra + (c - 3 - 6 * L)];
    }
    out[(p * group) * ldo + c] = v;
    if (group == 4) {
      out[(p * 4 + 1) * ldo + c] = t3[0];
      out[(p * 4 + 2) * ldo + c] = t3[1];
      out[(p * 4 + 3) * ldo + c] = t3[2];
    }
  }
}
}

extern "C" int sr_pe_embed(const float* x, int64_t P, int32_t L, const float* band_weights, const float* extra, int64_t ldextra,
                           int32_t E, const int64_t* extra_index, int32_t group, float* out, int64_t ldo, void* stream) {
  if (P < 0 || L < 0 || L > 16 || E < 0 || (group != 1 && group != 4) || ldo < 3 + 6 * L + E) return SR_EINVAL;
  if (P == 0) return SR_OK;
  if (!x || !out || (L > 0 && !band_weights) || (E > 0 && !extra)) return SR_EINVAL;
  sr_launch_stream(pe_embed_kernel, P * ldo, 256, stream, x, P, L, band_weights, extra, ldextra, E, extra_index, group, out, ldo);
  return sr_launch_status();
}

namespace {
__global__ __launch_bounds__(256) void pe_embed_bwd_kernel(const float* __restrict__ x, int64_t P, int L, const float* __restrict__ w,
                                                            int group, const float* __restrict__ gA0, int64_t ldg, float* __restrict__ xbar) {
  for (int64_t i = (int64_t)blockIdx.x * blockDim.x + threadIdx.x; i < P * 3; i += (int64_t)gridDim.x * blockDim.x) {
    const int64_t p = i / 3;
    const int c = (int)(i % 3);
    const float xv = x[i];
    const float* g0 = gA0 + (p * group) * ldg;
    const float* gt = group == 4 ? gA0 + (p * 4 + 1 + c) * ldg : nullptr;
    float acc = g0[c];
    for (int k = 0; k < L; ++k) {
      const float f = (float)(1 << k);
      float sn, cs;
      sincosf(xv * f, &sn, &cs);
      const float ws = w[2 * k], wc = w[2 * k + 1];
      const int is = 3 + 6 * k + c, ic = is + 3;
      acc += f * (ws * cs * g0[is] - wc * sn * g0[ic]);
      if (gt) acc -= f * f * (ws * sn * gt[is] + wc * cs * gt[ic]);
    }
    xbar[i] = acc;
  }
}
}

extern "C" int sr_pe_embed_bwd(const float* x, int64_t P, int32_t L, const float* band_weights, int32_t group, const float* gA0,
                               int64_t ldg, float* xbar, void* stream) {
  if (P < 0 || L < 0 || L > 16 || (group != 1 && group != 4) || ldg < 3 + 6 * L) return SR_EINVAL;
  if (P == 0) return SR_OK;
  if (!x || !gA0 || !xbar || (L > 0 && !band_weights)) return SR_EINVAL;
  sr_launch_stream(pe_embed_bwd_kernel, P * 3, 256, stream, x, P, L, band_weights, group, gA0, ldg, xbar);
  return sr_launch_status();
}
```

selfreconcode_amd/mlp_engine.py:

```python
import collections
import contextlib
import ctypes
import math
import os
import weakref
import torch

from . import _lib

ACT_NONE, ACT_SOFTPLUS100, ACT_RELU = _lib.SR_ACT_NONE, _lib.SR_ACT_SOFTPLUS100, _lib.SR_ACT_RELU
EPI_FWD, EPI_BWD = _lib.SR_EPI_FWD, _lib.SR_EPI_BWD

TN_SIDE_STREAM = True
GROUP_TN_BELOW = 16384
DEBUG_TN_DELAY_MS = int(os.environ.get("SR_DEBUG_TN_DELAY_MS", "0"))
_TN_STREAMS = {}
_TN_PENDING = set()
_DELAY_FLAG = {}

DEFERRED_PARAM_GRADS = False

_PACK_CACHE = {}
_ENTRY_BY_PTR = {}

_INPUT_GRADS_ONLY = False


def pad4(n):
    return (n + 3) // 4 * 4


class LayerSpec:
    __slots__ = ("K", "N", "act", "out_scale", "nfill")

    def __init__(self, K, N, act, out_scale=1.0, nfill=0):
        self.K, self.N, self.act, self.out_scale, self.nfill = K, N, act, float(out_scale), nfill


class MLPSpec:

    def __init__(self, layers, K0):
        self.layers = layers
        self.K0 = K0

    @staticmethod
    def sdf(multires=6, width=512, nlin=9, skip_in=(4,), d_out=257):
        K0 = 3 + 6 * multires
        layers = []
        k = K0
        for l in range(nlin):
            last = l == nlin - 1
            n = d_out if last else width
            if (l + 1) in skip_in:
                layers.append(LayerSpec(k, n - K0, ACT_SOFTPLUS100, 1.0 / math.sqrt(2.0), nfill=K0))
            else:
                layers.append(LayerSpec(k, n, ACT_NONE if last else ACT_SOFTPLUS100))
            k = n
        return MLPSpec(layers, K0)

    @staticmethod
    def relu_mlp(K0, widths):
        layers, k = [], K0
        for i, n in enumerate(widths):
            layers.append(LayerSpec(k, n, ACT_NONE if i == len(widths) - 1 else ACT_RELU))
            k = n
        return MLPSpec(layers, K0)


_GemmRecord = collections.namedtuple("_GemmRecord", "e0 e1 flop rows overlap N K mode group")


class _GemmProfile:

    def __init__(self):
        self.overlap = False
        self.reset(enabled=False)

    def reset(self, enabled, reserve=0):
        self.enabled = enabled
        self.records, self.chains, self.pool = [], [], []
        for _ in range(reserve if enabled else 0):
            e0, e1 = torch.cuda.Event(enable_timing=True), torch.cuda.Event(enable_timing=True)
            e0.record(); e1.record()
            self.pool.append((e0, e1))

    def pair(self):
        return self.pool.pop() if self.pool else (torch.cuda.Event(enable_timing=True), torch.cuda.Event(enable_timing=True))

    def launch(self, name, args, stream, timed=True, what=None, marks=None):
        if not (timed and self.enabled):
            _lib.call(name, ctypes.byref(args), stream)
            return
        e0, e1 = self.pair()
        e0.record()
        _lib.call(name, ctypes.byref(args), stream)
        e1.record()
        if marks is not None:
            marks.append((e0, e1) + what)
        else:
            rows, N, K, mode, group = what
            self.records.append(_GemmRecord(e0, e1, 2.0 * rows * N * K, rows, self.overlap, N, K, mode, group))

    def summary(self):
        if not self.records:
            return {"tflops": 0.0, "launches": 0, "avg_us": 0.0, "avg_flop": 0.0}
        torch.cuda.synchronize()
        for marks, live, overlap in self.chains:
            lv = live.tolist()
            for e0, e1, phase, fpr in marks:
                self.records.append(_GemmRecord(e0, e1, fpr * lv[phase], lv[phase], overlap, 0, 0, "chain", 1))
        self.chains = []
        times = [r.e0.elapsed_time(r.e1) for r in self.records]

        def rate(sel):
            f = sum(r.flop for r, t, k in zip(self.records, times, sel) if k)
            ms = sum(t for t, k in zip(times, sel) if k)
            n = sum(1 for k in sel if k)
            return (f / (ms * 1e-3) / 1e12 if ms > 0 else 0.0), n, (ms * 1e3 / n if n else 0.0), (f / n if n else 0.0)

        nt = [r.mode != "tn" for r in self.records]
        alone = [k and not r.overlap for k, r in zip(nt, self.records)]
        tf, n, us, fl = rate(alone)
        tf_all, n_all, us_all, _ = rate(nt)
        tf_big, n_big, _, _ = rate([a and r.rows >= 65536 for a, r in zip(alone, self.records)])
        tf_tn, n_tn, us_tn, _ = rate([not k for k in nt])
        self._times = times
        f_nt = float(sum(r.flop for r, k in zip(self.records, nt) if k))
        f_tn = float(sum(r.flop for r, k in zip(self.records, nt) if not k))
        return {"tflops": round(tf, 3), "launches": n, "avg_us": round(us, 3), "avg_flop": round(fl, 1), "tflops_large": round(tf_big, 3),
                "launches_large": n_big, "tflops_all": round(tf_all, 3), "launches_all": n_all, "avg_us_all": round(us_all, 3),
                "avg_flop_all": round(f_nt / max(n_all, 1), 1), "flops_total": f_nt, "flops_total_tn": f_tn,
                "tflops_tn": round(tf_tn, 3), "launches_tn": n_tn, "avg_us_tn": round(us_tn, 3)}

    def by_shape(self):
        if not self.records:
            return []
        times = getattr(self, "_times", None) or [r.e0.elapsed_time(r.e1) for r in self.records]
        acc = {}
        for r, t in zip(self.records, times):
            a = acc.setdefault((r.rows, r.N, r.K, r.mode, r.group, bool(r.overlap)), [0, 0.0, 0.0])
            a[0] += 1; a[1] += r.flop; a[2] += t
        rows = [{"M": k[0], "N": k[1], "K": k[2], "mode": k[3], "group": k[4], "overlap": k[5], "launches": v[0], "flop": v[1], "ms": round(v[2], 4),
                 "tflops": round(v[1] / (v[2] * 1e-3) / 1e12, 2) if v[2] > 0 else 0.0} for k, v in acc.items()]
        rows.sort(key=lambda r: -r["ms"])
        return rows


PROFILE = _GemmProfile()


def set_gemm_args(a, A, B, C, M, N, K, bias, group, act, mode, out_scale=1.0, aux=None, naux_fwd=0, nact_bwd=0, aux_scale=1.0, pitches=None):
    lda, ldb, ldc, ldaux = pitches or (A.stride(0), B.stride(0), C.stride(0), 0 if aux is None else aux.stride(0))
    a.A, a.lda, a.B, a.ldb, a.C, a.ldc = A.data_ptr(), lda, B.data_ptr(), ldb, C.data_ptr(), ldc
    a.M, a.N, a.K = M, N, K
    a.bias = _lib.ptr(bias)
    a.group, a.act, a.mode, a.out_scale = group, act, mode, out_scale
    a.aux, a.ldaux, a.naux_fwd, a.nact_bwd, a.aux_scale = _lib.ptr(aux), ldaux, naux_fwd, nact_bwd, aux_scale


def _gemm_nt(A, lda, B, ldb, C, ldc, M, N, K, bias, group, act, mode, out_scale=1.0, aux=None, ldaux=0, naux_fwd=0,
             nact_bwd=0, aux_scale=1.0):
    a = _lib.SrGemmArgs()
    set_gemm_args(a, A, B, C, M, N, K, bias, group, act, mode, out_scale, aux, naux_fwd, nact_bwd, aux_scale, (lda, ldb, ldc, ldaux))
    PROFILE.launch("sr_mlp_gemm_nt", a, _lib.stream_of(C), M >= 128 and N > 32, (M, N, K, mode, group))


_TnProblem = collections.namedtuple("_TnProblem", "Z ldz A lda R N K lddw group dW db accumulate")


def _tn_workspace(R, N, lddw):
    splits = ctypes.c_int32(0)
    ws = _lib.raw("sr_mlp_gemm_tn_workspace_floats")(R, N, lddw, ctypes.byref(splits))
    return max(int(ws), 1), splits.value


def _set_tn_args(a, Z, ldz, A, lda, R, N, K, lddw, group, dW, db, accumulate, partial, ws, splits):
    a.Z, a.ldz, a.A, a.lda, a.dW, a.lddw, a.partial = Z.data_ptr(), ldz, A.data_ptr(), lda, dW.data_ptr(), lddw, partial
    a.R, a.N, a.K, a.splits, a.accumulate = R, N, K, splits, 1 if accumulate else 0
    a.db, a.db_partial, a.group = db.data_ptr(), partial + 4 * ws, group


def _gemm_tn(Z, ldz, A, lda, R, N, K, lddw, group=1, dW=None, db=None, accumulate=False):
    ws, splits = _tn_workspace(R, N, lddw)
    if dW is None:
        dW = torch.empty((N, lddw), dtype=torch.float32, device=Z.device)
    partial = torch.empty((ws + splits * N,), dtype=torch.float32, device=Z.device)
    if db is None:
        db = torch.empty((N,), dtype=torch.float32, device=Z.device)
    a = _lib.SrGemmTnArgs()
    _set_tn_args(a, Z, ldz, A, lda, R, N, K, lddw, group, dW, db, accumulate, partial.data_ptr(), ws, splits)
    PROFILE.launch("sr_mlp_gemm_tn", a, _lib.stream_of(Z), R >= 128 and N > 32, (R, N, K, "tn", group))
    return dW, db


def _tn_is_narrow(N, lddw):
    return lddw <= 64 and N >= 256


def _gemm_tn_group(problems):
    problems = [_TnProblem(*p) for p in problems]
    g = _lib.SrGemmTnGroupArgs()
    g.n = len(problems)
    sizes, total = [], 0
    for p in problems:
        ws, splits = _tn_workspace(p.R, p.N, p.lddw)
        sizes.append((ws, splits, total))
        total += (ws + splits * p.N + 3) // 4 * 4
    partial = torch.empty((total,), dtype=torch.float32, device=problems[0].Z.device)
    for a, p, (ws, splits, off) in zip(g.p, problems, sizes):
        _set_tn_args(a, *p, partial.data_ptr() + 4 * off, ws, splits)
    _lib.call("sr_mlp_gemm_tn_group", ctypes.byref(g), _lib.stream_of(partial))


def _debug_delay(device, ms):
    f = _DELAY_FLAG.get(str(device))
    if f is None:
        f = _DELAY_FLAG[str(device)] = torch.zeros(2, dtype=torch.int32, device=device)
    _lib.call('sr_stream_flag_wait', f.data_ptr(), 0x40000000, 0, ms, torch.cuda.current_stream(device).cuda_stream)


def _tn_stream(device):
    key = str(device)
    st = _TN_STREAMS.get(key)
    if st is None:
        st = _TN_STREAMS[key] = torch.cuda.Stream(device=device)
    return st


def _launch_on_tn_stream(device, problems):
    main, side = torch.cuda.current_stream(device), _tn_stream(device)
    ready = torch.cuda.Event()
    ready.record(main)
    side.wait_event(ready)
    with torch.cuda.stream(side):
        if DEBUG_TN_DELAY_MS:
            _debug_delay(device, DEBUG_TN_DELAY_MS)
        if len(problems) == 1:
            p = problems[0]
            _gemm_tn(*p[:9], dW=p.dW, db=p.db, accumulate=p.accumulate)
        else:
            _gemm_tn_group(problems)
    for p in problems:
        p.Z.record_stream(side); p.A.record_stream(side)
    _TN_PENDING.add(str(device))


def join_weight_gradient_stream():
    for key in list(_TN_PENDING):
        st = _TN_STREAMS[key]
        torch.cuda.current_stream(st.device).wait_stream(st)
    _TN_PENDING.clear()


def _check_mat(t, name):
    if t.dtype != torch.float32 or not t.is_cuda or t.dim() != 2 or t.stride(1) != 1 or (t.stride(0) % 4) or (t.data_ptr() % 16):
        raise RuntimeError(f"mlp_engine: {name} must be a GPU fp32 matrix with unit column stride, row pitch % 4 == 0 "
                           f"and 16-byte alignment (got {tuple(t.shape)}, strides {t.stride()}, {t.dtype}, {t.device})")


def _bias_segments(b0, R, group):
    if b0 is None or b0.dim() != 2:
        return None
    S = b0.shape[0]
    if S < 1 or R % S or (R // S) % group or b0.stride(1) != 1:
        raise RuntimeError(f"mlp_engine: segmented first-layer bias {tuple(b0.shape)} does not divide {R} rows of group {group}")
    return S, R // S


def forward(spec, A0, Ws, bs, group):
    _check_mat(A0, "A0")
    R = A0.shape[0]
    acts, X = [], A0
    seg = _bias_segments(bs[0], R, group)
    with _lib.on_device(A0.device):
        for l, L in enumerate(spec.layers):
            _check_mat(Ws[l], f"W{l}")
            C = torch.empty((R, pad4(L.N + L.nfill)), dtype=torch.float32, device=A0.device)
            if l == 0 and seg is not None:
                S, rs = seg
                for s in range(S):
                    Xs, Cs = X[s * rs:(s + 1) * rs], C[s * rs:(s + 1) * rs]
                    _gemm_nt(Xs, X.stride(0), Ws[l], Ws[l].stride(0), Cs, C.stride(0), rs, L.N, L.K, bs[0][s], group, L.act, EPI_FWD,
                             out_scale=L.out_scale, aux=A0[s * rs:(s + 1) * rs] if L.nfill else None, ldaux=A0.stride(0), naux_fwd=L.nfill)
            else:
                _gemm_nt(X, X.stride(0), Ws[l], Ws[l].stride(0), C, C.stride(0), R, L.N, L.K, bs[l], group, L.act, EPI_FWD,
                         out_scale=L.out_scale, aux=A0 if L.nfill else None, ldaux=A0.stride(0), naux_fwd=L.nfill)
            acts.append(C)
            X = C
    return acts


_DW_GROUPED, _DW_SIDE, _DW_SINK, _DW_SEGMENTED, _DW_AUTOGRAD = range(5)


def _weight_gradient_route(l, L, Ws, bs, seg, grouped):
    segmented = l == 0 and seg is not None
    sink = None
    if DEFERRED_PARAM_GRADS and Ws is not None:
        if not segmented:
            sink = _deferred_sink(Ws[l], bs[l])
        if sink is None and not Ws[l].requires_grad:
            e = _ENTRY_BY_PTR.get(Ws[l].data_ptr())
            if e is not None and any(r() is not None and r().requires_grad for r in e.src):
                raise RuntimeError("mlp_engine: a packed weight handed out without autograd node (deferred mode) met a layer call "
                                   "that has no deferred sink (bias that is not the layer's own leaf parameter?): its gradient would be lost")
    if sink is None:
        return (_DW_SEGMENTED if segmented else _DW_AUTOGRAD), None
    if grouped is not None and not _tn_is_narrow(L.N, pad4(L.K)) and len(grouped) < _lib.SR_TN_GROUP_MAX:
        return _DW_GROUPED, sink
    if TN_SIDE_STREAM and not PROFILE.enabled:
        return _DW_SIDE, sink
    return _DW_SINK, sink


def reverse(spec, A0, WTs, acts, Ybar, group, need_input_grad=True, need_param_grad=True, Ws=None, bs=None):
    _check_mat(Ybar, "Ybar")
    R = A0.shape[0]
    nl = len(spec.layers)
    dWs, dbs = [None] * nl, [None] * nl
    A0bar_extra = None
    Zbar = Ybar
    A0bar = None
    seg = _bias_segments(bs[0], R, group) if bs is not None else None
    grouped = [] if (0 < R < GROUP_TN_BELOW and TN_SIDE_STREAM and not PROFILE.enabled) else None
    with _lib.on_device(A0.device):
        for l in range(nl - 1, -1, -1):
            L = spec.layers[l]
            X = A0 if l == 0 else acts[l - 1]
            if need_param_grad:
                route, sink = _weight_gradient_route(l, L, Ws, bs, seg, grouped)
                if sink is not None:
                    p = _TnProblem(Zbar, Zbar.stride(0), X, X.stride(0), R, L.N, L.K, pad4(L.K), group, *sink)
                    if route == _DW_GROUPED:
                        grouped.append(p)
                    elif route == _DW_SIDE:
                        _launch_on_tn_stream(A0.device, [p])
                    else:
                        _gemm_tn(*p[:9], dW=p.dW, db=p.db, accumulate=p.accumulate)
                elif route == _DW_SEGMENTED:
                    S, rs = seg
                    dWs[0] = torch.empty((L.N, pad4(L.K)), dtype=torch.float32, device=A0.device)
                    dbs[0] = torch.zeros((S, L.N), dtype=torch.float32, device=A0.device)
                    for s in range(S):
                        _gemm_tn(Zbar[s * rs:(s + 1) * rs], Zbar.stride(0), X[s * rs:(s + 1) * rs], X.stride(0), rs, L.N, L.K, pad4(L.K), group,
                                 dW=dWs[0], db=dbs[0][s], accumulate=s > 0)
                else:
                    dWs[l], dbs[l] = _gemm_tn(Zbar, Zbar.stride(0), X, X.stride(0), R, L.N, L.K, pad4(L.K), group)
            if l > 0:
                Pv = spec.layers[l - 1]
                Znew = torch.empty((R, pad4(L.K)), dtype=torch.float32, device=A0.device)
                _gemm_nt(Zbar, Zbar.stride(0), WTs[l], WTs[l].stride(0), Znew, Znew.stride(0), R, L.K, L.N, None, group, Pv.act,
                         EPI_BWD, out_scale=Pv.out_scale, aux=acts[l - 1], ldaux=acts[l - 1].stride(0), nact_bwd=Pv.N,
                         aux_scale=Pv.out_scale)
                if Pv.nfill and need_input_grad:
                    A0bar_extra = Znew[:, Pv.N:Pv.N + Pv.nfill]
                Zbar = Znew
            elif need_input_grad:
                A0bar = torch.empty((R, pad4(L.K)), dtype=torch.float32, device=A0.device)
                _gemm_nt(Zbar, Zbar.stride(0), WTs[0], WTs[0].stride(0), A0bar, A0bar.stride(0), R, L.K, L.N, None, 1, ACT_NONE,
                         EPI_FWD)
                if A0bar_extra is not None:
                    A0bar[:, :A0bar_extra.shape[1]] += A0bar_extra
        if grouped:
            _launch_on_tn_stream(A0.device, grouped)
    return A0bar, dWs, dbs


def transpose_padded(W, K):
    N = W.shape[0]
    WT = torch.zeros((K, pad4(N)), dtype=W.dtype, device=W.device)
    WT[:, :N] = W[:, :K].t()
    return WT


def pad_cols(t, width):
    if t.shape[1] == width and t.is_contiguous():
        return t
    return torch.nn.functional.pad(t, (0, width - t.shape[1]))


def rows_pad(a, width, b=None, pair=False):
    ref = a if a is not None else b
    R = ref.shape[0]
    if not pair and a.shape[1] == width and a.stride(1) == 1 and a.stride(0) % 4 == 0 and a.data_ptr() % 16 == 0:
        return a
    srcs = []
    for t in (a, b):
        if t is not None and (t.stride(1) != 1 or t.dtype != torch.float32):
            t = t.contiguous().float()
        srcs.append(t)
    a, b = srcs
    out = torch.empty((R * (2 if pair else 1), width), dtype=torch.float32, device=ref.device)
    with _lib.on_device(ref.device):
        _lib.call("sr_rows_pad", _lib.ptr(a), 0 if a is None else a.stride(0), 0 if a is None else min(a.shape[1], width),
                  _lib.ptr(b), 0 if b is None else b.stride(0), 0 if b is None else min(b.shape[1], width),
                  R, 2 if pair else 1, _lib.ptr(out), width, width, _lib.stream_of(ref))
    return out


def rows_frame_sum(X, index, n):
    P, E = X.shape
    if X.dtype != torch.float32 or X.stride(1) != 1:
        X = X.float().contiguous()
    index = index.contiguous()
    out = torch.empty((n, E), dtype=torch.float32, device=X.device)
    part = _lib.workspace("sr_rows_frame_sum_workspace_floats", P, E, n, device=X.device, dtype=torch.float32)
    with _lib.on_device(X.device):
        _lib.call("sr_rows_frame_sum", _lib.ptr(X), X.stride(0), P, E, _lib.ptr(index), n, _lib.ptr(part), _lib.ptr(out), _lib.stream_of(X))
    return out


@contextlib.contextmanager
def input_grads_only():
    global _INPUT_GRADS_ONLY
    prev = _INPUT_GRADS_ONLY
    _INPUT_GRADS_ONLY = True
    try:
        yield
    finally:
        _INPUT_GRADS_ONLY = prev


class MLPCoreFunction(torch.autograd.Function):

    @staticmethod
    def forward(ctx, spec, A0, *wb):
        nl = len(spec.layers)
        Ws, bs = list(wb[:nl]), list(wb[nl:])
        acts = forward(spec, A0, Ws, bs, 1)
        ctx.spec = spec
        ctx.save_for_backward(A0, *wb, *acts[:-1])
        ctx.set_materialize_grads(False)
        NL = spec.layers[-1].N
        out = acts[-1]
        return out if out.shape[1] == NL else out[:, :NL]

    @staticmethod
    def backward(ctx, ybar):
        if ybar is None:
            return (None,) * (2 + 2 * len(ctx.spec.layers))
        saved = ctx.saved_tensors
        nl = len(ctx.spec.layers)
        A0, wb, acts = saved[0], saved[1:1 + 2 * nl], saved[1 + 2 * nl:]
        need_par = any(ctx.needs_input_grad[2:]) and not _INPUT_GRADS_ONLY
        outs = MLPCoreBackward.apply(ctx.spec, ctx.needs_input_grad[1], need_par, A0, ybar, *wb, *acts)
        return (None,) + tuple(outs)


class MLPCoreBackward(torch.autograd.Function):

    @staticmethod
    def forward(ctx, spec, need_in, need_par, A0, ybar, *rest):
        nl = len(spec.layers)
        Ws, bs, acts = list(rest[:nl]), list(rest[nl:2 * nl]), list(rest[2 * nl:])
        NL = spec.layers[-1].N
        yb = rows_pad(ybar, pad4(NL))
        WTs = [transposed_of(Ws[l], spec.layers[l].K) for l in range(nl)]
        A0bar, dWs, dbs = reverse(spec, A0, WTs, acts, yb, 1, need_in, need_par, Ws, bs)
        ctx.spec = spec
        ctx.save_for_backward(A0, ybar, *Ws, *bs)
        ctx.set_materialize_grads(False)
        if not need_par:
            dWs, dbs = [None] * nl, [None] * nl
        if A0bar is not None and A0bar.shape[1] != A0.shape[1]:
            A0bar = rows_pad(A0bar[:, :spec.K0], A0.shape[1])
        return (A0bar,) + tuple(dWs) + tuple(dbs)

    @staticmethod
    def backward(ctx, U, *param_cots):
        spec = ctx.spec
        nl = len(spec.layers)
        if any(c is not None for c in param_cots):
            raise NotImplementedError("selfreconcode_amd: differentiating MLP parameter gradients again is not supported "
                                      "(the reference only differentiates input gradients, network.py:102-114)")
        n_in = 5 + 2 * nl + (nl - 1)
        if U is None:
            return (None,) * n_in
        saved = ctx.saved_tensors
        A0, ybar = saved[0], saved[1]
        Ws, bs = list(saved[2:2 + nl]), list(saved[2 + nl:2 + 2 * nl])
        NL = spec.layers[-1].N
        R = A0.shape[0]
        A0i = rows_pad(A0, A0.shape[1], U, pair=True)
        acts2 = forward(spec, A0i, Ws, bs, 2)
        ydot = acts2[-1].view(R, 2, -1)[:, 1, :NL]
        ybi = rows_pad(None, pad4(NL), ybar, pair=True)
        WTs = [transposed_of(Ws[l], spec.layers[l].K) for l in range(nl)]
        need_in = ctx.needs_input_grad[3]
        need_par = any(ctx.needs_input_grad[5:5 + 2 * nl])
        A0bar2, dWs, dbs = reverse(spec, A0i, WTs, acts2, ybi, 2, need_in, need_par, Ws, bs)
        gA0 = A0bar2.view(R, 2, -1)[:, 0, :] if A0bar2 is not None else None
        if gA0 is not None and gA0.shape[1] != A0.shape[1]:
            gA0 = rows_pad(gA0[:, :spec.K0], A0.shape[1])
        return (None, None, None, gA0, ydot.contiguous()) + tuple(dWs) + tuple(dbs) + (None,) * (nl - 1)


def mlp_apply(spec, A0, Ws, bs):
    return MLPCoreFunction.apply(spec, A0, *Ws, *bs)


class _Pack:
    __slots__ = ("W", "WT", "norms", "sig", "src", "bias_param", "dW", "db", "bias", "fresh", "dirty")

    def __init__(self, W, WT, norms):
        self.W, self.WT, self.norms, self.sig, self.src = W, WT, norms, None, ()
        self.dW = self.db = self.bias = self.bias_param = None
        self.fresh, self.dirty = True, False


def _sig(*ts):
    return tuple((t.data_ptr(), t._version, tuple(t.shape)) for t in ts)


def _lin_params(lin):
    return (lin.weight_v, lin.weight_g) if hasattr(lin, "weight_g") else (lin.weight, None)


def _lin_sig(v, g):
    return _sig(v) if g is None else _sig(v, g)


def _raise_if_dirty(e):
    if e.dirty:
        raise RuntimeError("mlp_engine: parameters changed while deferred gradients were pending; call flush_param_grads() "
                           "before the optimizer step")


def _drop_entry(key):
    e = _PACK_CACHE.pop(key, None)
    if e is not None:
        _ENTRY_BY_PTR.pop(e.W.data_ptr(), None)


def _pack_entry(key, sig, build, owner=None):
    e = _PACK_CACHE.get(key)
    if e is None and owner is not None:
        weakref.finalize(owner, _drop_entry, key)
    if e is None or e.sig != sig:
        if e is not None:
            _raise_if_dirty(e)
            _drop_entry(key)
        e = build()
        e.sig = sig
        _PACK_CACHE[key] = e
        _ENTRY_BY_PTR[e.W.data_ptr()] = e
    return e


class PackWeightNorm(torch.autograd.Function):
    @staticmethod
    def forward(ctx, v, g):
        K = v.shape[1]

        def build():
            with torch.no_grad():
                w, norms = torch._weight_norm_interface(v, g, 0)
                W = pad_cols(w, pad4(K)).contiguous()
                return _Pack(W, transpose_padded(W, K), norms)
        e = _pack_entry(id(v), _sig(v, g), build, owner=v)
        e.src = (weakref.ref(v), weakref.ref(g))
        ctx.save_for_backward(v, g, e.norms)
        ctx.set_materialize_grads(False)
        return e.W.detach()

    @staticmethod
    def backward(ctx, gW):
        if gW is None:
            return None, None
        v, g, norms = ctx.saved_tensors
        gv, gg = torch.ops.aten._weight_norm_interface_backward(gW[:, :v.shape[1]].contiguous(), v, g, norms, 0)
        return gv, gg


class PackPlain(torch.autograd.Function):
    @staticmethod
    def forward(ctx, w):
        K = w.shape[1]

        def build():
            with torch.no_grad():
                W = pad_cols(w, pad4(K)).contiguous()
                if W.data_ptr() == w.data_ptr():
                    W = W.clone()
                return _Pack(W, transpose_padded(W, K), None)
        e = _pack_entry(id(w), _sig(w), build, owner=w)
        e.src = (weakref.ref(w),)
        ctx.K = K
        ctx.set_materialize_grads(False)
        return e.W.detach()

    @staticmethod
    def backward(ctx, gW):
        return None if gW is None else gW[:, :ctx.K]


def refresh_packs(lins):
    if not lins or not _lin_params(lins[0])[0].is_cuda:
        return
    stale = []
    for lin in lins:
        v, g = _lin_params(lin)
        e = _PACK_CACHE.get(id(v))
        if e is None:
            continue
        sig = _lin_sig(v, g)
        if e.sig != sig:
            _raise_if_dirty(e)
            if e.W.shape != (v.shape[0], pad4(v.shape[1])):
                continue
            stale.append((e, v, g, sig))
    for i in range(0, len(stale), _lib.SR_PACK_MAX_LAYERS):
        chunk = stale[i:i + _lib.SR_PACK_MAX_LAYERS]
        t = _lib.SrPackTable()
        t.nlayers = len(chunk)
        for j, (e, v, g, sig) in enumerate(chunk):
            L = t.layer[j]
            vv = v.detach()
            if not vv.is_contiguous():
                vv = vv.contiguous()
            L.v, L.g = _lib.ptr(vv), (0 if g is None else _lib.ptr(g.detach().contiguous()))
            L.W, L.WT, L.norms = _lib.ptr(e.W), _lib.ptr(e.WT), (0 if g is None else _lib.ptr(e.norms))
            L.N, L.K, L.ldw, L.ldwt = v.shape[0], v.shape[1], e.W.stride(0), e.WT.stride(0)
        with _lib.on_device(chunk[0][1].device), torch.no_grad():
            _lib.call("sr_pack_weights", ctypes.byref(t), _lib.stream_of(chunk[0][1]))
        for e, v, g, sig in chunk:
            e.sig = sig
        torch.autograd.graph.increment_version([t for e, _, _, _ in chunk for t in (e.W, e.WT, e.norms) if t is not None])


def pack_linear(lin):
    v, g = _lin_params(lin)
    if DEFERRED_PARAM_GRADS:
        e = _PACK_CACHE.get(id(v))
        b = lin.bias
        if e is not None and e.sig == _lin_sig(v, g) and e.src and b is not None and b.is_leaf and b.requires_grad:
            e.bias_param = b
            return e.W
    W = PackPlain.apply(v) if g is None else PackWeightNorm.apply(v, g)
    e = _ENTRY_BY_PTR.get(W.data_ptr())
    if e is not None:
        e.bias_param = lin.bias
    return W


def packed_weights_of(module, nlayers):
    d = module.__dict__
    mods = module._modules
    lins = [mods["lin" + str(l)] for l in range(nlayers)]
    params = []
    for lin in lins:
        P = lin._parameters
        v = P.get('weight_v')
        if v is not None:
            params.append(v); params.append(P['weight_g'])
        else:
            params.append(P['weight'])
        b = P.get('bias')
        if b is not None:
            params.append(b)
    key = (DEFERRED_PARAM_GRADS,) + tuple((id(p), p.data_ptr(), p._version, p.requires_grad) for p in params)
    hit = d.get('_sr_packs')
    if hit is not None and hit[0] == key:
        return list(hit[1]), list(hit[2])
    refresh_packs(lins)
    Ws, bs = [pack_linear(lin) for lin in lins], [lin.bias for lin in lins]
    if DEFERRED_PARAM_GRADS and all(W.grad_fn is None and not W.requires_grad and W.data_ptr() in _ENTRY_BY_PTR for W in Ws):
        d['_sr_packs'] = (key, list(Ws), list(bs))
    else:
        d.pop('_sr_packs', None)
    return Ws, bs


def transposed_of(W, K):
    e = _ENTRY_BY_PTR.get(W.data_ptr())
    if e is not None:
        WT = e.WT
        if WT.shape == (K, pad4(W.shape[0])):
            return WT
        if W.stride(0) == e.W.stride(0) and W.shape[0] <= e.W.shape[0] and K <= WT.shape[0] and pad4(W.shape[0]) <= WT.shape[1]:
            return WT[:K, :pad4(W.shape[0])]
    return transpose_padded(W, K)


def set_deferred_param_grads(flag):
    global DEFERRED_PARAM_GRADS
    flush_param_grads()
    DEFERRED_PARAM_GRADS = bool(flag)


def _deferred_sink(W, b):
    e = _ENTRY_BY_PTR.get(W.data_ptr())
    if e is None or b is None or not b.requires_grad or W.shape[0] > e.W.shape[0] or W.stride(0) != e.W.stride(0):
        return None
    n, full = W.shape[0], W.shape[0] == e.W.shape[0]
    if full:
        if not b.is_leaf:
            return None
    else:
        base = e.bias_param
        if base is None or not base.is_leaf or not base.requires_grad or b.data_ptr() != base.data_ptr():
            return None
        b = base
    if e.dW is None:
        e.dW = torch.empty_like(e.W)
        e.db = torch.empty((e.W.shape[0],), dtype=torch.float32, device=e.W.device)
        e.fresh = True
    if e.fresh and not full:
        e.dW.zero_(); e.db.zero_()
        e.fresh = False
    accumulate = not e.fresh
    e.fresh = False
    e.dirty = True
    e.bias = b
    return e.dW[:n], e.db[:n], accumulate


def flush_param_grads(only=None):
    todo = [e for e in _PACK_CACHE.values() if e.dirty and (only is None or id(e.src[0]()) in only)]
    if not todo:
        return
    join_weight_gradient_stream()
    for i in range(0, len(todo), _lib.SR_PACK_MAX_LAYERS):
        chunk = todo[i:i + _lib.SR_PACK_MAX_LAYERS]
        t = _lib.SrUnpackTable()
        t.nlayers = len(chunk)
        outs = []
        for j, e in enumerate(chunk):
            L = t.layer[j]
            src = tuple(r() for r in e.src)
            v = src[0]
            g = src[1] if len(src) == 2 else None
            acc = v.grad is not None and (g is None or g.grad is not None)
            gv = v.grad if acc else torch.empty_like(v, memory_format=torch.contiguous_format)
            gg = None
            if g is not None:
                gg = g.grad if acc else torch.empty_like(g, memory_format=torch.contiguous_format)
            if acc and (not gv.is_contiguous() or (gg is not None and not gg.is_contiguous())):
                acc = False
                gv = torch.empty_like(v, memory_format=torch.contiguous_format)
                gg = None if g is None else torch.empty_like(g, memory_format=torch.contiguous_format)
            vd = v.detach()
            if not vd.is_contiguous():
                vd = vd.contiguous()
            L.dW, L.lddw = _lib.ptr(e.dW), e.dW.stride(0)
            L.v, L.g, L.norms = _lib.ptr(vd), (0 if g is None else _lib.ptr(g.detach().contiguous())), (0 if g is None else _lib.ptr(e.norms))
            L.gv, L.gg, L.N, L.K, L.accumulate = _lib.ptr(gv), _lib.ptr(gg), v.shape[0], v.shape[1], 1 if acc else 0
            b = e.bias
            fold_bias = b.grad is not None and b.grad.is_contiguous() and b.grad.dtype == torch.float32
            L.db, L.gb = (_lib.ptr(e.db), _lib.ptr(b.grad)) if fold_bias else (0, 0)
            outs.append((e, v, g, gv, gg, acc, vd, fold_bias))
        dev = chunk[0].W.device
        with _lib.on_device(dev), torch.no_grad():
            _lib.call("sr_unpack_grads", ctypes.byref(t), torch.cuda.current_stream(dev).cuda_stream)
        for e, v, g, gv, gg, acc, _, fold_bias in outs:
            if not acc:
                v.grad = gv if v.grad is None else v.grad.add_(gv)
                if g is not None:
                    g.grad = gg if g.grad is None else g.grad.add_(gg)
            b = e.bias
            if fold_bias:
                torch.autograd.graph.increment_version(b.grad)
            elif b.grad is None:
                b.grad = e.db
                e.db = torch.empty_like(e.db)
            else:
                b.grad.add_(e.db)
            e.fresh = True
            e.dirty = False
```

selfreconcode_amd/model/Deformer.py:

```python
import ctypes
import os

import numpy as np
import torch
import torch.nn as nn
import torch.nn.functional as F

from .. import _lib
from .Embedder import embed_rows
from ..MCAcc.grid_sampler_mine import GridSamplerMine3dFunction
from ..mlp_engine import MLPSpec, mlp_apply, pad_cols, pad4, pack_linear
from ..utils.utils import resolve_band_weights


BATCH_FRAMES = True
HOIST_FRAME_CODE = True


_EYE3 = {}


def _eye3(device):
    e = _EYE3.get(device)
    if e is None:
        e = _EYE3[device] = torch.eye(3).to(device)
        if e.is_cuda:
            torch.cuda.current_stream(device).synchronize()
    return e


class CompositeDeformer(nn.Module):
    def __init__(self, deformers):
        super().__init__()
        self.N = len(deformers)
        self.defs = nn.ModuleList(deformers)

    def forward(self, ps, conds, batch_inds=None, **kwargs):
        assert self.N == len(conds)
        out = ps
        for cond, deformer in zip(conds, self.defs):
            out = deformer(out, cond, batch_inds, **kwargs)
        return out


class MLPTranslator(nn.Module):

    def __init__(self, feature_vector_size, multires, weight_norm=False):
        super().__init__()
        assert multires > 0
        dims = [3 + 6 * multires + feature_vector_size, 512, 512, 512, 512, 3]
        self.feature_vector_size = feature_vector_size
        self.multires = multires
        self.num_layers = len(dims)
        for l in range(0, self.num_layers - 1):
            lin = nn.Linear(dims[l], dims[l + 1])
            if weight_norm:
                print('MLPTranslator:weight norm can influence weight initialization, can not produce small weights as '
                      'initialization. Now do not use weight_norm')
            if l == self.num_layers - 2:
                torch.nn.init.normal_(lin.weight, mean=0., std=0.001)
                torch.nn.init.constant_(lin.bias, 0.)
            setattr(self, "lin" + str(l), lin)
        self.spec = MLPSpec.relu_mlp(dims[0], dims[1:])
        self.offset = None

    def packed_weights(self):
        from ..mlp_engine import packed_weights_of
        return packed_weights_of(self, len(self.spec.layers))

    def hoisted_first_layer(self, conds, frames=None):
        npe = 3 + 6 * self.multires
        W0 = self.lin0.weight
        Bf = conds.reshape(-1, self.feature_vector_size) @ W0[:, npe:].t() + self.lin0.bias
        if frames is not None and Bf.shape[0] != frames:
            raise ValueError(f"MLPTranslator: {Bf.shape[0]} condition codes for a batch of {frames} frames")
        W0p = pad_cols(W0[:, :npe], pad4(npe))
        spec = getattr(self, "_spec_pe", None)
        if spec is None:
            spec = self._spec_pe = MLPSpec.relu_mlp(npe, [L.N for L in self.spec.layers])
        return spec, W0p, Bf

    def forward(self, ps, conds, batch_inds=None, **kwargs):
        ratio = kwargs['ratio']['deformerRatio']
        ws = resolve_band_weights(self.multires, ratio)
        if batch_inds is None and HOIST_FRAME_CODE and ps.dim() == 3:
            spec, W0p, Bf = self.hoisted_first_layer(conds, ps.shape[0])
            Ws, bs = self.packed_weights()
            if BATCH_FRAMES:
                A0 = embed_rows(ps.reshape(-1, 3), self.multires, ws)
                self.offset = mlp_apply(spec, A0, [W0p] + Ws[1:], [Bf] + bs[1:]).view(ps.shape[0], ps.shape[1], 3)
                return ps[..., :3] + self.offset
            outs = []
            for p_f, B_f in zip(ps.unbind(0), Bf.unbind(0)):
                A0 = embed_rows(p_f, self.multires, ws)
                outs.append(mlp_apply(spec, A0, [W0p] + Ws[1:], [B_f] + bs[1:]))
            self.offset = torch.stack(outs, 0)
            return ps[..., :3] + self.offset
        if batch_inds is not None:
            flat, index, seg = ps, batch_inds, 0
        else:
            nb, nv = ps.shape[0], ps.shape[1]
            flat = ps.reshape(-1, 3)
            index = torch.arange(nb, device=ps.device).repeat_interleave(nv)
            seg = nv
        A0 = embed_rows(flat, self.multires, ws, extra=conds.reshape(-1, self.feature_vector_size), extra_index=index, segment=seg)
        Ws, bs = self.packed_weights()
        x = mlp_apply(self.spec, A0, Ws, bs)
        if batch_inds is not None:
            self.offset = x
            return ps[..., :3] + x
        self.offset = x.view(ps.shape[0], ps.shape[1], 3)
        return ps[..., :3] + self.offset


def getTranslatorNet(device, conf):
    return MLPTranslator(conf.get_int('condlen'), multires=conf.get_int('multires')).to(device)


def batch_rodrigues(theta):
    angle = torch.norm(theta + 1e-8, p=2, dim=1, keepdim=True)
    axis = theta / angle
    half = angle * 0.5
    q = torch.cat([torch.cos(half), torch.sin(half) * axis], dim=1)
    q = q / q.norm(p=2, dim=1, keepdim=True)
    w, x, y, z = q[:, 0], q[:, 1], q[:, 2], q[:, 3]
    w2, x2, y2, z2 = w * w, x * x, y * y, z * z
    wx, wy, wz, xy, xz, yz = w * x, w * y, w * z, x * y, x * z, y * z
    return torch.stack([w2 + x2 - y2 - z2, 2 * xy - 2 * wz, 2 * wy + 2 * xz,
                        2 * wz + 2 * xy, w2 - x2 + y2 - z2, 2 * yz - 2 * wx,
                        2 * xz - 2 * wy, 2 * wx + 2 * yz, w2 - x2 - y2 + z2], dim=1).view(-1, 3, 3)


def _tree_levels(parents):
    depth = [0] * len(parents)
    for i in range(1, len(parents)):
        depth[i] = depth[int(parents[i])] + 1
    return [[i for i in range(len(parents)) if depth[i] == d] for d in range(1, max(depth) + 1)]


class LBSkinner(nn.Module):

    def __init__(self, ws, bmins, bmaxs, Js, parents, init_pose=None, align_corners=False):
        super().__init__()

        def as_row(v):
            if isinstance(v, list):
                return torch.tensor(v, dtype=torch.float).view(1, 3)
            if isinstance(v, np.ndarray):
                return torch.from_numpy(v.astype(np.float32)).view(1, 3)
            return v.view(1, 3)
        self.register_buffer('b_min', as_row(bmins))
        self.register_buffer('b_max', as_row(bmaxs))
        ws = torch.from_numpy(ws.astype(np.float32)) if isinstance(ws, np.ndarray) else ws.to(torch.float)
        assert ws.dim() == 5 and ws.shape[0] == 1 and ws.shape[1] == 24
        self.register_buffer('ws', ws.contiguous(memory_format=torch.channels_last_3d))
        assert align_corners is False
        self.align_corners = align_corners
        self.register_buffer('Js', Js.view(24, 3).float())
        self.parents = [int(p) for p in parents]
        self._levels = _tree_levels(self.parents)
        if init_pose is None:
            raise NotImplementedError("the reference always builds the skinner with an init pose (network.py:843,851)")
        if isinstance(init_pose, np.ndarray):
            init_pose = torch.from_numpy(init_pose.astype(np.float32))
        if init_pose.numel() == 24 * 3:
            self.init_pose_inverse(batch_rodrigues(init_pose.view(-1, 3)).view(24, 3, 3), self.Js)
        else:
            self.register_buffer('init_pose', init_pose.view(24, 4, 4))

    def _apply(self, fn, *a, **k):
        out = super()._apply(fn, *a, **k)
        if not self.ws.is_contiguous(memory_format=torch.channels_last_3d):
            self.ws = self.ws.contiguous(memory_format=torch.channels_last_3d)
        return out

    def init_pose_inverse(self, init_pose, Js):
        R, T = [init_pose[0]], [Js[0]]
        for i in range(1, 24):
            pa = self.parents[i]
            R.append(R[pa] @ init_pose[i])
            T.append(R[pa] @ (Js[i] - Js[pa]) + T[pa])
        inv = torch.zeros(24, 4, 4)
        for i in range(24):
            inv[i, :3, :3] = R[i].t()
            inv[i, :3, 3] = -(R[i].t() @ T[i])
            inv[i, 3, 3] = 1.
        self.register_buffer('init_pose', inv)

    def _chain(self, poses):
        B = poses.shape[0]
        R = batch_rodrigues(poses.reshape(-1, 3)).view(B, 24, 3, 3)
        rel = self.Js.clone()
        rel[1:] = self.Js[1:] - self.Js[self.parents[1:]]
        local = torch.cat([torch.cat([R, rel.view(1, 24, 3, 1).expand(B, 24, 3, 1)], 3),
                           torch.cat([rel.new_zeros(3), rel.new_ones(1)]).view(1, 1, 1, 4).expand(B, 24, 1, 4)], 2)
        G = [None] * 24
        G[0] = local[:, 0]
        for level in self._levels:
            pa = torch.stack([G[self.parents[i]] for i in level], 1)
            prod = pa @ local[:, level]
            for n, i in enumerate(level):
                G[i] = prod[:, n]
        return torch.stack(G, 1)

    def _buffers_key(self):
        return tuple((t.data_ptr(), t._version) for t in (self.Js, self.init_pose, self.b_min, self.b_max))

    def _host_consts(self):
        key = self._buffers_key()
        if getattr(self, "_hc_key", None) != key:
            js = (ctypes.c_float * 72)(*self.Js.detach().cpu().view(-1).tolist())
            pa = (ctypes.c_int32 * 24)(*[max(p, 0) if i else 0 for i, p in enumerate(self.parents)])
            ip = (ctypes.c_float * 384)(*self.init_pose.detach().cpu().view(-1).tolist())
            self._hc = (js, pa, ip)
            self._box = (self.b_min.view(-1).tolist(), self.b_max.view(-1).tolist())
            self._hc_key = key
        return self._hc

    def _box_consts(self):
        self._host_consts()
        return self._box

    def posed_chain(self, poses):
        if poses.is_cuda:
            return _PosedChain.apply(self, poses)
        G = self._chain(poses)
        return G, G @ self.init_pose.view(1, 24, 4, 4)

    def posed_transforms(self, poses):
        return self.posed_chain(poses)[1]

    def posedSkeleton(self, conds):
        poses, trans = conds
        assert poses.shape[0] == trans.shape[0]
        return self.posed_chain(poses)[0][:, :, :3, 3]

    def fill_lbs_fields(self, a, A, trans):
        A12 = A[:, :, :3, :].contiguous()
        vol = self.ws.permute(0, 2, 3, 4, 1)
        assert vol.is_contiguous()
        a.A, a.trans, a.nframes = _lib.ptr(A12), _lib.ptr(trans), A.shape[0]
        a.vol, a.D, a.H, a.W = _lib.ptr(vol), vol.shape[1], vol.shape[2], vol.shape[3]
        box = self._box_consts()
        for i in range(3):
            a.bmin[i], a.bmax[i] = box[0][i], box[1][i]
        return A12, vol

    def _lbs_args(self, flat, A, trans, batch_inds, ppf, tp=None):
        a = _lib.SrLbsArgs()
        keep = self.fill_lbs_fields(a, A, trans)
        a.p, a.tp, a.P = _lib.ptr(flat), _lib.ptr(tp), flat.shape[0]
        a.batch_inds, a.points_per_frame = _lib.ptr(batch_inds), ppf
        return a, keep

    def fused(self, ps, A, trans, batch_inds=None, with_jac=False, tps=None):
        flat = ps.reshape(-1, 3).contiguous()
        P = flat.shape[0]
        tr = trans.contiguous()
        tp = None if tps is None else tps.reshape(-1, 3).contiguous()
        ppf = 0 if batch_inds is not None else (ps.shape[1] if ps.dim() == 3 else P)
        a, keep = self._lbs_args(flat, A, tr, batch_inds, ppf, tp)
        y = torch.empty_like(flat)
        jac = torch.empty((P, 3, 3), device=flat.device) if with_jac else None
        a.y, a.jac = _lib.ptr(y), _lib.ptr(jac)
        _lib.launch("sr_lbs_fwd", flat, ctypes.byref(a))
        return y.view(ps.shape), jac

    def forward(self, ps, conds, batch_inds=None, **kwargs):
        if type(ps) == list:
            tps, ps = ps
        else:
            tps = ps
        poses, trans = conds
        batch_size = poses.shape[0]
        assert batch_size == trans.shape[0]
        A = self.posed_transforms(poses)
        needs_graph = torch.is_grad_enabled() and (ps.requires_grad or tps.requires_grad or poses.requires_grad or trans.requires_grad)
        if not needs_graph:
            y, _ = self.fused(ps, A, trans, batch_inds, False, None if tps is ps else tps)
            return y
        if tps is ps:
            flat = ps.reshape(-1, 3)
            ppf = 0 if batch_inds is not None else ps.shape[1]
            y = _FusedLBS.apply(self, flat, A, trans, batch_inds, ppf)
            return y.view(ps.shape)
        return self._composite(ps, tps, A, trans, batch_inds)

    def _composite(self, ps, tps, A, trans, batch_inds):
        batch_size = A.shape[0]
        nps = 2. * (tps.reshape(-1, 3) - self.b_min) / (self.b_max - self.b_min) - 1.
        w = GridSamplerMine3dFunction.apply(self.ws, nps.reshape(1, 1, 1, -1, 3)).view(24, -1).transpose(0, 1)
        A12 = A[:, :, :3, :].reshape(batch_size, 24, 12)
        if batch_inds is None:
            nb, pnum, _ = ps.shape
            assert nb == batch_size
            T = torch.matmul(w.view(nb, pnum, 24), A12).view(nb, pnum, 3, 4)
            return (T[..., :3] @ ps.unsqueeze(-1)).squeeze(-1) + T[..., 3] + trans.view(-1, 1, 3)
        p = ps.reshape(-1, 3)
        Tall = (w @ A12.permute(1, 0, 2).reshape(24, batch_size * 12)).view(-1, batch_size, 12)
        T = torch.gather(Tall, 1, batch_inds.view(-1, 1, 1).expand(-1, 1, 12)).view(-1, 3, 4)
        return (T[..., :3] @ p.unsqueeze(-1)).squeeze(-1) + T[..., 3] + trans[batch_inds]

    def fused_backward(self, flat, A, batch_inds, ppf, ybar, need_p, need_A, need_t, Jbar=None):
        N, dev = A.shape[0], flat.device
        a, keep = self._lbs_args(flat, A, None, batch_inds, ppf)
        cots = [None if ybar is None else ybar.contiguous().float()] + ([] if Jbar is None else [Jbar.contiguous().float()])
        pbar = torch.empty_like(flat) if need_p else None
        Abar = torch.empty((N, 24, 12), device=dev) if need_A else None
        tbar = torch.empty((N, 3), device=dev) if (need_t and ybar is not None) else None
        part = _lib.workspace("sr_lbs_bwd_workspace_floats", flat.shape[0], N, device=dev, dtype=torch.float32)
        _lib.launch("sr_lbs_bwd" if Jbar is None else "sr_lbs_jac_bwd", flat, ctypes.byref(a), *cots, pbar, Abar, tbar, part)
        return pbar, Abar, tbar


def _frame_major(flat, A, batch_inds):
    return flat if batch_inds is not None else flat.view(A.shape[0], -1, 3)


def _cotangent_4x4(Abar):
    return None if Abar is None else F.pad(Abar.view(-1, 24, 3, 4), (0, 0, 0, 1))


class _PosedChain(torch.autograd.Function):
    @staticmethod
    def forward(ctx, skin, poses):
        p = poses.detach().contiguous().float().view(-1, 24, 3)
        B = p.shape[0]
        G = torch.empty((B, 24, 4, 4), dtype=torch.float32, device=p.device)
        A = torch.empty_like(G)
        js, pa, ip = skin._host_consts()
        _lib.launch("sr_lbs_chain_fwd", p, p, B, js, pa, ip, G, A)
        ctx.skin = skin
        ctx.save_for_backward(p)
        ctx.pshape = poses.shape
        ctx.set_materialize_grads(False)
        return G, A

    @staticmethod
    def backward(ctx, Gbar, Abar):
        if Gbar is None and Abar is None:
            return None, None
        (p,) = ctx.saved_tensors
        js, pa, ip = ctx.skin._host_consts()
        out = torch.empty_like(p)
        gb = None if Gbar is None else Gbar.contiguous().float()
        ab = None if Abar is None else Abar.contiguous().float()
        _lib.launch("sr_lbs_chain_bwd", p, p, p.shape[0], js, pa, ip, ab, gb, out)
        return None, out.view(ctx.pshape)


class _FusedLBS(torch.autograd.Function):

    @staticmethod
    def forward(ctx, skin, flat, A, trans, batch_inds, ppf):
        flat = flat.contiguous()
        y, _ = skin.fused(_frame_major(flat, A, batch_inds), A, trans, batch_inds, False, None)
        ctx.skin, ctx.ppf = skin, ppf
        ctx.save_for_backward(flat, A, trans, batch_inds)
        return y.reshape(-1, 3)

    @staticmethod
    def backward(ctx, ybar):
        flat, A, trans, batch_inds = ctx.saved_tensors
        skin = ctx.skin
        need_p, need_A, need_t = ctx.needs_input_grad[1], ctx.needs_input_grad[2], ctx.needs_input_grad[3]
        if torch.is_grad_enabled():
            ps = _frame_major(flat, A, batch_inds)
            y2 = skin._composite(ps, ps, A, trans, batch_inds).reshape(-1, 3)
            ins = [t for t, n in ((flat, need_p), (A, need_A), (trans, need_t)) if n]
            gs = list(torch.autograd.grad(y2, ins, ybar, create_graph=True, allow_unused=True))
            out = [gs.pop(0) if n else None for n in (need_p, need_A, need_t)]
            return None, out[0], out[1], out[2], None, None
        pbar, Abar, tbar = skin.fused_backward(flat, A, batch_inds, ctx.ppf, ybar, need_p, need_A, need_t)
        return None, pbar, _cotangent_4x4(Abar), tbar, None, None


class _LBSValueJacobian(torch.autograd.Function):

    @staticmethod
    def forward(ctx, skin, q, A, trans, batch_inds, ppf):
        flat = q.reshape(-1, 3).contiguous().float()
        y, J = skin.fused(_frame_major(flat, A, batch_inds), A, trans, batch_inds, True, None)
        ctx.skin, ctx.ppf = skin, ppf
        ctx.save_for_backward(flat, A, batch_inds)
        ctx.set_materialize_grads(False)
        return y.reshape(-1, 3), J

    @staticmethod
    def backward(ctx, ybar, Jbar):
        flat, A, batch_inds = ctx.saved_tensors
        skin = ctx.skin
        if ybar is None and Jbar is None:
            return (None,) * 6
        need_q, need_A, need_t = ctx.needs_input_grad[1], ctx.needs_input_grad[2], ctx.needs_input_grad[3]
        Jb = torch.zeros((flat.shape[0], 3, 3), device=flat.device) if Jbar is None else Jbar
        qbar, Abar, tbar = skin.fused_backward(flat, A, batch_inds, ctx.ppf, ybar, need_q, need_A, need_t, Jb)
        return None, qbar, _cotangent_4x4(Abar), tbar, None, None


def deformer_value_jacobian(deformer, ps, defconds, batch_inds, ratio):
    tr, skin = deformer.defs[0], deformer.defs[1]
    d_cond, (poses, trans) = defconds[0], defconds[1]
    q, Jq = translator_value_jacobian(tr, ps, d_cond, batch_inds, ratio)
    A = skin.posed_transforms(poses)
    y, Jl = _LBSValueJacobian.apply(skin, q, A, trans, batch_inds, 0)
    from ..utils.utils import small_matmul
    return y, small_matmul(Jl, Jq)


def is_fused_composite(deformer):
    return (isinstance(deformer, CompositeDeformer) and deformer.N == 2 and isinstance(deformer.defs[0], MLPTranslator)
            and isinstance(deformer.defs[1], LBSkinner))


class TranslatorValueJacobian(torch.autograd.Function):

    @staticmethod
    def forward(ctx, tr, ratio, x, conds, index, segment, spec, *wb):
        from .. import mlp_engine as me
        from .Embedder import band_weight_tensor
        spec = spec or tr.spec
        nl = len(spec.layers)
        Ws, bs = list(wb[:nl]), list(wb[nl:])
        flat = x.reshape(-1, 3).contiguous().float()
        P = flat.shape[0]
        wt, _ = band_weight_tensor(resolve_band_weights(tr.multires, ratio), tr.multires, flat.device)
        E = 0 if conds is None else tr.feature_vector_size
        ldo = me.pad4(3 + 6 * tr.multires + E)
        A0 = torch.empty((P * 4, ldo), dtype=torch.float32, device=flat.device)
        cd = None if conds is None else conds.reshape(-1, E).contiguous().float()
        with _lib.on_device(flat.device):
            _lib.launch("sr_pe_embed", flat, flat, P, tr.multires, wt, cd, 0 if cd is None else cd.stride(0), E, index, 4, A0, ldo)
            acts = me.forward(spec, A0, Ws, bs, 4)
        out = acts[-1].view(P, 4, -1)[:, :, :3]
        d = flat + out[:, 0]
        J = out[:, 1:4].transpose(1, 2) + _eye3(flat.device)
        ctx.tr, ctx.wt, ctx.segment, ctx.n_extra, ctx.xshape, ctx.spec, ctx.E = tr, wt, segment, 0 if cd is None else cd.shape[0], x.shape, spec, E
        ctx.set_materialize_grads(False)
        ctx.save_for_backward(flat, index, A0, *wb, *acts[:-1])
        return d.view(x.shape), J

    @staticmethod
    def backward(ctx, dbar, Jbar):
        from .. import mlp_engine as me
        tr, spec = ctx.tr, ctx.spec
        nl = len(spec.layers)
        saved = ctx.saved_tensors
        flat, index, A0 = saved[0], saved[1], saved[2]
        wb, acts = saved[3:3 + 2 * nl], list(saved[3 + 2 * nl:])
        Ws = list(wb[:nl])
        P = flat.shape[0]
        if dbar is None and Jbar is None:
            return (None,) * (7 + 2 * nl)
        ybar = torch.zeros((P, 4, 4), dtype=torch.float32, device=flat.device)
        if dbar is not None:
            ybar[:, 0, :3] = dbar.reshape(-1, 3)
        if Jbar is not None:
            ybar[:, 1:4, :3] = Jbar.transpose(1, 2)
        WTs = [me.transposed_of(Ws[l], spec.layers[l].K) for l in range(nl)]
        acts_full = acts + [None]
        need_par = any(ctx.needs_input_grad[7:])
        need_x = ctx.needs_input_grad[2]
        need_in = need_x or (ctx.needs_input_grad[3] and ctx.E > 0)
        A0bar, dWs, dbs = me.reverse(spec, A0, WTs, acts_full, ybar.view(P * 4, 4), 4, need_in, need_par, Ws, list(wb[nl:]))
        if not need_par:
            dWs, dbs = [None] * nl, [None] * nl
        xbar = None
        if need_x:
            xbar = torch.empty_like(flat)
            _lib.launch("sr_pe_embed_bwd", flat, flat, P, tr.multires, ctx.wt, 4, A0bar, A0bar.stride(0), xbar)
            if dbar is not None:
                xbar = xbar + dbar.reshape(-1, 3)
            xbar = xbar.view(ctx.xshape)
        gcond = None
        if ctx.needs_input_grad[3] and ctx.E:
            E = ctx.E
            ge = A0bar.view(P, 4, -1)[:, 0, 3 + 6 * tr.multires:3 + 6 * tr.multires + E]
            if ctx.segment:
                gcond = ge.reshape(ctx.n_extra, ctx.segment, E).sum(1)
            else:
                gcond = (me.rows_frame_sum(ge, index, ctx.n_extra) if ctx.n_extra <= 32
                         else torch.zeros((ctx.n_extra, E), dtype=ge.dtype, device=ge.device).index_add(0, index, ge))
        return (None, None, xbar, gcond, None, None, None) + tuple(dWs) + tuple(dbs)


def translator_value_jacobian(tr, ps, conds, batch_inds, ratio):
    r = ratio['deformerRatio'] if isinstance(ratio, dict) else ratio
    if batch_inds is not None:
        index, seg = batch_inds, 0
    else:
        index = torch.arange(ps.shape[0], device=ps.device).repeat_interleave(ps.shape[1])
        seg = ps.shape[1]
    Ws, bs = tr.packed_weights()
    if batch_inds is None and HOIST_FRAME_CODE and ps.dim() == 3:
        spec, W0p, Bf = tr.hoisted_first_layer(conds, ps.shape[0])
        if BATCH_FRAMES:
            return TranslatorValueJacobian.apply(tr, r, ps.contiguous(), None, None, 0, spec, W0p, *Ws[1:], Bf, *bs[1:])
        ds_, Js_ = [], []
        for p_f, B_f in zip(ps.unbind(0), Bf.unbind(0)):
            d_f, J_f = TranslatorValueJacobian.apply(tr, r, p_f.contiguous(), None, None, 0, spec, W0p, *Ws[1:], B_f, *bs[1:])
            ds_.append(d_f); Js_.append(J_f)
        return torch.stack(ds_, 0), torch.cat(Js_, 0)
    return TranslatorValueJacobian.apply(tr, r, ps, conds, index, seg, None, *Ws, *bs)


def smooth_weights(weights, times=3):
    from .. import ops
    _lib.require_gpu(weights)
    if weights.dim() != 5 or weights.shape[0] != 1:
        raise ValueError(f"smooth_weights: weights [1,nj,D,H,W] expected, got {tuple(weights.shape)}")
    if int(times) <= 0:
        return weights
    return ops.lbsw_smooth(weights.detach()[0].contiguous().float(), times).unsqueeze(0)


def _three(v):
    if torch.is_tensor(v):
        v = v.detach().cpu().numpy()
    return [float(x) for x in np.asarray(v, dtype=np.float32).reshape(3)]


def compute_lbswField(bmins, bmaxs, resolutions, smpl_verts, smpl_ws, align_corners=False, mean_neighbor=5, smooth_times=30):
    from .. import ops
    _lib.require_gpu(smpl_verts, smpl_ws)
    field = ops.lbsw_knn_blend(smpl_verts, smpl_ws, _three(bmins), _three(bmaxs), resolutions, mean_neighbor, align_corners)
    return ops.lbsw_smooth(field, smooth_times, consume=True).unsqueeze(0)


LBS_BOX_MARGIN = (0.15, 0.15, 0.20)


def initialLBSkinner(gender, shape, pose, resolution, bmins=None, bmaxs=None, smpl=None):
    from ..smpl_pytorch import getSMPL
    _lib.require_gpu(shape, pose)
    smpl = (smpl if smpl is not None else getSMPL(gender)).to(shape.device)
    Js = smpl.skeleton(shape.view(1, -1), True)[0]
    verts = smpl(shape.view(1, -1), pose.view(1, 24, 3), True)[0][0]
    skinner = initial_lbs_skinner(verts, smpl.weight[0], Js.view(24, 3), smpl.parents, pose.view(24, 3), resolution, bmins, bmaxs)
    return skinner, verts, smpl.faces_tensor.to(verts.device)


def initial_lbs_skinner(verts, skin_weights, Js, parents, init_pose, resolution, bmins=None, bmaxs=None):
    _lib.require_gpu(verts, skin_weights)
    if bmins is None or bmaxs is None:
        margin = np.array(LBS_BOX_MARGIN, dtype=np.float32)
        bmins = (verts.min(0)[0].cpu().numpy() - margin).tolist()
        bmaxs = (verts.max(0)[0].cpu().numpy() + margin).tolist()
    ws = compute_lbswField(bmins, bmaxs, resolution, verts, skin_weights, align_corners=False, mean_neighbor=30, smooth_times=30)
    pose = torch.from_numpy(init_pose.astype(np.float32)) if isinstance(init_pose, np.ndarray) else init_pose.detach().float().cpu()
    skinner = LBSkinner(ws, _three(bmins), _three(bmaxs), torch.as_tensor(Js).detach().float().cpu(), np.asarray(parents), init_pose=pose,
                        align_corners=False)
    return skinner.to(verts.device)
```

Before: 23.40.

## Skip primal rows in deformer reverse sweep when only Jacobian cotangent flows

When the deformer backward receives only a Jacobian cotangent (no displacement gradient), no input gradient is needed, and all layers are ReLU or linear, the reverse sweep now carries only the 3 tangent rows per sample instead of 4. The NT epilogue reads the ReLU mask from the primal row of the saved activations, and the TN weight-gradient kernel maps tangent rows to their group-of-4 activation rows with a 24-row step. The bias gradient is dropped in this path because primal rows carry a zero cotangent. This removes about a quarter of the backward GEMM work for that case, at the cost of extra kernel variants and strided activation reads.

```diff
diff --git a/include/selfrecon_hip.h b/include/selfrecon_hip.h
--- a/include/selfrecon_hip.h
+++ b/include/selfrecon_hip.h
@@ -72,6 +72,7 @@
   int32_t naux_fwd;
   int32_t nact_bwd;
   float aux_scale;
+  int32_t tangent_rows;
 } sr_gemm_args;
 int sr_mlp_gemm_nt(const sr_gemm_args* host_args, void* stream);
 int sr_mlp_gemm_nt_tile(int32_t M, int32_t ncols, int32_t* bm_out, int32_t* bn_out);
@@ -93,6 +94,7 @@
   float* partial;
   int32_t R, N, K, splits, accumulate;
   float* db; float* db_partial; int32_t group;
+  int32_t tangent_rows;
 } sr_gemm_tn_args;
 int64_t sr_mlp_gemm_tn_workspace_floats(int32_t R, int32_t N, int64_t lddw, int32_t* host_splits_out);
 int sr_mlp_gemm_tn(const sr_gemm_tn_args* host_args, void* stream);
diff --git a/selfreconcode_amd/csrc/mlp_gemm.hip b/selfreconcode_amd/csrc/mlp_gemm.hip
--- a/selfreconcode_amd/csrc/mlp_gemm.hip
+++ b/selfreconcode_amd/csrc/mlp_gemm.hip
@@ -36,6 +36,10 @@
   d = x < 1e-3f ? x * (1.0f - x * (0.5f - x * 0.16666667f)) : 1.0f - em;
   c2 = 100.0f * em;
 }
+
+constexpr int TRB = 24;
+__device__ __forceinline__ int tangent_primal_row(int c) { return 4 * (int)((unsigned)c / 3u); }
+__device__ __forceinline__ int tangent_group4_row(int c) { const int s = (int)((unsigned)c / 3u); return c + s + 1; }
 
 template <int WM, int WN, int TM, int TN>
 struct Cfg {
@@ -97,7 +101,7 @@
   }
 };
 
-template <int WM, int WN, int TM, int TN, int G>
+template <int WM, int WN, int TM, int TN, int G, bool TR = false>
 __device__ __forceinline__ void epilogue(const sr_gemm_args& g, f32x16 (&acc)[TM][TN], int m0, int n0, int wm, int wn,
                                          int li, int kh, float* __restrict__ stage) {
   constexpr int SP = TN * 32 + 4;
@@ -136,6 +140,13 @@
           if (col >= g.nact_bwd) {
 #pragma unroll
             for (int j = 0; j < 4; ++j) o[j] = v[j] * g.out_scale;
+          } else if constexpr (TR) {
+#pragma unroll
+            for (int j = 0; j < 4; ++j) {
+              float d = 1.f;
+              if (g.act == SR_ACT_RELU && r0 + j < g.M) d = g.aux[(int64_t)tangent_primal_row(r0 + j) * g.ldaux + col] > 0.f ? 1.f : 0.f;
+              o[j] = d * g.aux_scale * v[j];
+            }
           } else {
             float sv[4];
 #pragma unroll
@@ -186,7 +197,7 @@
   }
 }
 
-template <int WM, int WN, int TM, int TN, int G, int MODE, int ACT>
+template <int WM, int WN, int TM, int TN, int G, int MODE, int ACT, bool TR = false>
 __device__ __forceinline__ void epilogue_interior(const sr_gemm_args& g, f32x16 (&acc)[TM][TN], int m0, int n0, int wm, int wn, int li,
                                                   int kh, float* __restrict__ stage) {
   constexpr int SP = TN * 32 + 4;
@@ -212,6 +223,14 @@
             else { o[s] = z * os; }
 #pragma unroll
             for (int tI = 1; tI < G; ++tI) o[s + tI] = d * v[s + tI] * os;
+          }
+        } else if constexpr (TR) {
+          static_assert(!TR || (G == 1 && ACT != SR_ACT_SOFTPLUS100), "tangent rows: ReLU / linear layers, one row at a time");
+#pragma unroll
+          for (int j = 0; j < 4; ++j) {
+            float d = 1.f;
+            if constexpr (ACT == SR_ACT_RELU) d = g.aux[(int64_t)tangent_primal_row(r0 + j) * g.ldaux + col] > 0.f ? 1.f : 0.f;
+            o[j] = d * as * v[j];
           }
         } else {
           float sv[4];
@@ -256,6 +275,12 @@
   if (g.act == SR_ACT_SOFTPLUS100) epilogue_interior<WM, WN, TM, TN, G, MODE, SR_ACT_SOFTPLUS100>(g, acc, m0, n0, wm, wn, li, kh, stage);
   else if (g.act == SR_ACT_RELU) epilogue_interior<WM, WN, TM, TN, G, MODE, SR_ACT_RELU>(g, acc, m0, n0, wm, wn, li, kh, stage);
   else epilogue_interior<WM, WN, TM, TN, G, MODE, SR_ACT_NONE>(g, acc, m0, n0, wm, wn, li, kh, stage);
+}
+template <int WM, int WN, int TM, int TN>
+__device__ __forceinline__ void epilogue_interior_tangent_rows(const sr_gemm_args& g, f32x16 (&acc)[TM][TN], int m0, int n0, int wm, int wn, int li,
+                                                               int kh, float* __restrict__ stage) {
+  if (g.act == SR_ACT_RELU) epilogue_interior<WM, WN, TM, TN, 1, SR_EPI_BWD, SR_ACT_RELU, true>(g, acc, m0, n0, wm, wn, li, kh, stage);
+  else epilogue_interior<WM, WN, TM, TN, 1, SR_EPI_BWD, SR_ACT_NONE, true>(g, acc, m0, n0, wm, wn, li, kh, stage);
 }
 
 struct NoProbe { __device__ __forceinline__ void operator()(int) const {} };
@@ -363,7 +388,10 @@
 
   float* stage = smem + wave * (TM * 32 * (TN * 32 + 4));
   const bool interior = m0 + C_::BM <= g.M && n0 + C_::BN <= (g.mode == SR_EPI_FWD ? g.N : (g.nact_bwd < g.N ? g.nact_bwd : g.N));
-  if (interior) {
+  if (g.tangent_rows) {
+    if (interior) epilogue_interior_tangent_rows<WM, WN, TM, TN>(g, acc, m0, n0, wm, wn, li, kh, stage);
+    else epilogue<WM, WN, TM, TN, 1, true>(g, acc, m0, n0, wm, wn, li, kh, stage);
+  } else if (interior) {
     if (g.mode == SR_EPI_FWD) {
       switch (g.group) {
         case 1: epilogue_interior_act<WM, WN, TM, TN, 1, SR_EPI_FWD>(g, acc, m0, n0, wm, wn, li, kh, stage); break;
@@ -438,42 +466,55 @@
   const float* zcol = g.Z + (n0 + cqz < zmax ? n0 + cqz : zmax);
   const float* xcol = g.A + (k0 + cqx < xmax ? k0 + cqx : xmax);
   f32x4 rz[TLZ], rx[TLX];
+  const bool tangent = g.tangent_rows != 0;
+  const int xrow0 = tangent ? r_begin / 3 * 4 : r_begin, xrows = tangent ? g.R / 3 * 4 : g.R;
   const __amdgpu_buffer_rsrc_t zrsrc = sr_make_rsrc(g.Z + (int64_t)r_begin * g.ldz, (int64_t)(g.R - r_begin) * g.ldz * 4);
-  const __amdgpu_buffer_rsrc_t xrsrc = sr_make_rsrc(g.A + (int64_t)r_begin * g.lda, (int64_t)(g.R - r_begin) * g.lda * 4);
+  const __amdgpu_buffer_rsrc_t xrsrc = sr_make_rsrc(g.A + (int64_t)xrow0 * g.lda, (int64_t)(xrows - xrow0) * g.lda * 4);
   uint32_t zbyte[TLZ], xbyte[TLX];
 #pragma unroll
   for (int j = 0; j < TLZ; ++j) zbyte[j] = (uint32_t)(((int64_t)(lrz + j * (256 / ZT)) * g.ldz + (zcol - g.Z)) * 4);
 #pragma unroll
-  for (int j = 0; j < TLX; ++j) xbyte[j] = (uint32_t)(((int64_t)(lrx + j * (256 / XT)) * g.lda + (xcol - g.A)) * 4);
-  const int last_full = r_end - TBR;
-  auto load = [&](int r0, auto tail) {
+  for (int j = 0; j < TLX; ++j) {
+    const int row = lrx + j * (256 / XT);
+    xbyte[j] = (uint32_t)(((int64_t)(tangent ? tangent_group4_row(row) : row) * g.lda + (xcol - g.A)) * 4);
+  }
+#define SR_TN_STEP_CONSTANTS(tan)                                                                                              \
+  [[maybe_unused]] constexpr int RB = decltype(tan)::value ? TRB : TBR;                                                        \
+  [[maybe_unused]] constexpr int NLZ = (RB * ZT + 255) / 256, NLX = (RB * XT + 255) / 256, NHS = RB / 4;                       \
+  static_assert(NLZ <= TLZ && NLX <= TLX && (RB * ZT) % 256 == 0, "loader passes")
+  auto load = [&](int r0, auto tail, auto tan) {
+    SR_TN_STEP_CONSTANTS(tan);
     if constexpr (decltype(tail)::value) {
 #pragma unroll
-      for (int j = 0; j < TLZ; ++j) {
+      for (int j = 0; j < NLZ; ++j) {
         int gr = r0 + lrz + j * (256 / ZT);
         gr = gr < r_end ? gr : r_end - 1;
         rz[j] = *reinterpret_cast<const f32x4*>(zcol + (int64_t)gr * g.ldz);
       }
 #pragma unroll
-      for (int j = 0; j < TLX; ++j) {
+      for (int j = 0; j < NLX; ++j) {
         int gr = r0 + lrx + j * (256 / XT);
         gr = gr < r_end ? gr : r_end - 1;
+        if constexpr (decltype(tan)::value) gr = tangent_group4_row(gr);
         rx[j] = *reinterpret_cast<const f32x4*>(xcol + (int64_t)gr * g.lda);
       }
     } else {
+      const int last_full = r_end - RB;
       const int rc = r0 < last_full ? r0 : last_full;
-      const uint32_t zo = (uint32_t)((int64_t)(rc - r_begin) * g.ldz * 4), xo = (uint32_t)((int64_t)(rc - r_begin) * g.lda * 4);
-#pragma unroll
-      for (int j = 0; j < TLZ; ++j) rz[j] = sr_buffer_load16(zrsrc, zbyte[j], zo);
-#pragma unroll
-      for (int j = 0; j < TLX; ++j) rx[j] = sr_buffer_load16(xrsrc, xbyte[j], xo);
+      const int xr = decltype(tan)::value ? (rc - r_begin) / 3 * 4 : rc - r_begin;
+      const uint32_t zo = (uint32_t)((int64_t)(rc - r_begin) * g.ldz * 4), xo = (uint32_t)((int64_t)xr * g.lda * 4);
+#pragma unroll
+      for (int j = 0; j < NLZ; ++j) rz[j] = sr_buffer_load16(zrsrc, zbyte[j], zo);
+#pragma unroll
+      for (int j = 0; j < NLX; ++j) rx[j] = sr_buffer_load16(xrsrc, xbyte[j], xo);
     }
   };
-  auto store = [&](int buf, int r0, auto tail) {
+  auto store = [&](int buf, int r0, auto tail, auto tan) {
+    SR_TN_STEP_CONSTANTS(tan);
     float* zs = Zs(buf);
     float* xs = Xs(buf);
 #pragma unroll
-    for (int j = 0; j < TLZ; ++j) {
+    for (int j = 0; j < NLZ; ++j) {
       const int row = lrz + j * (256 / ZT);
       f32x4 z = rz[j];
       if constexpr (decltype(tail)::value) {
@@ -483,7 +524,7 @@
       *reinterpret_cast<f32x4*>(zs + row * C::ZLD + cqz) = z;
     }
 #pragma unroll
-    for (int j = 0; j < TLX; ++j) {
+    for (int j = 0; j < NLX; ++j) {
       const int row = lrx + j * (256 / XT);
       f32x4 x = rx[j];
       if constexpr (decltype(tail)::value) {
@@ -498,18 +539,20 @@
   typedef float f32x2 __attribute__((ext_vector_type(2)));
   float z0a[HS], z1a[HS], x0a[HS], x1a[HS], z0b[HS], z1b[HS], x0b[HS], x1b[HS];
   const int zoff = kh * C::ZLD + wm * 64 + 2 * li, xoff = kh * C::XLD + wn * 64 + 2 * li;
-  auto read_half = [&](int buf, int half, float (&z0)[HS], float (&z1)[HS], float (&x0)[HS], float (&x1)[HS]) {
-    const float* zb = Zs(buf) + zoff + half * HS * 2 * C::ZLD;
-    const float* xb = Xs(buf) + xoff + half * HS * 2 * C::XLD;
-#pragma unroll
-    for (int e = 0; e < HS; ++e) {
+  auto read_half = [&](int buf, int half, float (&z0)[HS], float (&z1)[HS], float (&x0)[HS], float (&x1)[HS], auto tan) {
+    SR_TN_STEP_CONSTANTS(tan);
+    const float* zb = Zs(buf) + zoff + half * NHS * 2 * C::ZLD;
+    const float* xb = Xs(buf) + xoff + half * NHS * 2 * C::XLD;
+#pragma unroll
+    for (int e = 0; e < NHS; ++e) {
       const f32x2 z = *reinterpret_cast<const f32x2*>(zb + 2 * e * C::ZLD), x = *reinterpret_cast<const f32x2*>(xb + 2 * e * C::XLD);
       z0[e] = z.x; z1[e] = z.y; x0[e] = x.x; x1[e] = x.y;
     }
   };
-  auto mfma_half = [&](const float (&z0)[HS], const float (&z1)[HS], const float (&x0)[HS], const float (&x1)[HS]) {
-#pragma unroll
-    for (int e = 0; e < HS; ++e) {
+  auto mfma_half = [&](const float (&z0)[HS], const float (&z1)[HS], const float (&x0)[HS], const float (&x1)[HS], auto tan) {
+    SR_TN_STEP_CONSTANTS(tan);
+#pragma unroll
+    for (int e = 0; e < NHS; ++e) {
       acc[0][0] = __builtin_amdgcn_mfma_f32_32x32x2f32(z0[e], x0[e], acc[0][0], 0, 0, 0);
       acc[0][1] = __builtin_amdgcn_mfma_f32_32x32x2f32(z0[e], x1[e], acc[0][1], 0, 0, 0);
       acc[1][0] = __builtin_amdgcn_mfma_f32_32x32x2f32(z1[e], x0[e], acc[1][0], 0, 0, 0);
@@ -527,31 +570,33 @@
       else { bsum0 += z0[e]; bsum1 += z1[e]; }
     }
   };
-  const int nsteps = (r_end - r_begin + TBR - 1) / TBR;
-  auto run = [&](auto tail, auto bias) {
-    load(r_begin, tail);
-    store(0, r_begin, tail);
-    load(r_begin + TBR, tail);
+  const int step_rows = tangent ? TRB : TBR;
+  const int nsteps = (r_end - r_begin + step_rows - 1) / step_rows;
+  auto run = [&](auto tail, auto bias, auto tan) {
+    SR_TN_STEP_CONSTANTS(tan);
+    load(r_begin, tail, tan);
+    store(0, r_begin, tail, tan);
+    load(r_begin + RB, tail, tan);
     __syncthreads();
-    read_half(0, 0, z0a, z1a, x0a, x1a);
+    read_half(0, 0, z0a, z1a, x0a, x1a, tan);
     for (int t = 0; t < nsteps; ++t) {
       const int cur = t & 1;
-      store(cur ^ 1, r_begin + (t + 1) * TBR, tail);
-      load(r_begin + (t + 2) * TBR, tail);
-      read_half(cur, 1, z0b, z1b, x0b, x1b);
-      mfma_half(z0a, z1a, x0a, x1a);
-#pragma unroll
-      for (int i = 0; i < TLZ + TLX; ++i) {
+      store(cur ^ 1, r_begin + (t + 1) * RB, tail, tan);
+      load(r_begin + (t + 2) * RB, tail, tan);
+      read_half(cur, 1, z0b, z1b, x0b, x1b, tan);
+      mfma_half(z0a, z1a, x0a, x1a, tan);
+#pragma unroll
+      for (int i = 0; i < NLZ + NLX; ++i) {
         __builtin_amdgcn_sched_group_barrier(0x200, 1, 0);
         __builtin_amdgcn_sched_group_barrier(0x008, 1, 0);
       }
 #pragma unroll
-      for (int i = 0; i < TLZ + TLX; ++i) {
+      for (int i = 0; i < NLZ + NLX; ++i) {
         __builtin_amdgcn_sched_group_barrier(0x020, 1, 0);
         __builtin_amdgcn_sched_group_barrier(0x008, 1, 0);
       }
 #pragma unroll
-      for (int i = 0; i < HS; ++i) {
+      for (int i = 0; i < NHS; ++i) {
         __builtin_amdgcn_sched_group_barrier(0x100, 1, 0);
         __builtin_amdgcn_sched_group_barrier(0x008, 1, 0);
       }
@@ -559,19 +604,22 @@
       if constexpr (decltype(bias)::value) bias_half(z0a, z1a);
       __builtin_amdgcn_sched_barrier(0);
       __syncthreads();
-      read_half(cur ^ 1, 0, z0a, z1a, x0a, x1a);
+      read_half(cur ^ 1, 0, z0a, z1a, x0a, x1a, tan);
       __builtin_amdgcn_sched_barrier(0);
-      mfma_half(z0b, z1b, x0b, x1b);
+      mfma_half(z0b, z1b, x0b, x1b, tan);
       if constexpr (decltype(bias)::value) bias_half(z0b, z1b);
       __builtin_amdgcn_sched_barrier(0);
     }
   };
+#undef SR_TN_STEP_CONSTANTS
   if (nsteps > 0) {
-    const bool tail = ((r_end - r_begin) % TBR) != 0;
-    if (tail) {
-      if (do_bias) run(std::true_type{}, std::true_type{}); else run(std::true_type{}, std::false_type{});
+    const bool tail = ((r_end - r_begin) % step_rows) != 0;
+    if (tangent) {
+      if (tail) run(std::true_type{}, std::false_type{}, std::true_type{}); else run(std::false_type{}, std::false_type{}, std::true_type{});
+    } else if (tail) {
+      if (do_bias) run(std::true_type{}, std::true_type{}, std::false_type{}); else run(std::true_type{}, std::false_type{}, std::false_type{});
     } else {
-      if (do_bias) run(std::false_type{}, std::true_type{}); else run(std::false_type{}, std::false_type{});
+      if (do_bias) run(std::false_type{}, std::true_type{}, std::false_type{}); else run(std::false_type{}, std::false_type{}, std::false_type{});
     }
   }
   __syncthreads();
@@ -657,7 +705,8 @@
     } else {
       const int n = (int)(i - quads);
       float s = 0.f;
-      for (int p = 0; p < splits; ++p) s += db_partial[(int64_t)p * N + n];
+      if (db_partial)
+        for (int p = 0; p < splits; ++p) s += db_partial[(int64_t)p * N + n];
       db[n] = (accumulate ? db[n] : 0.f) + s;
     }
   }
@@ -711,7 +760,9 @@
   if ((a->naux_fwd > 0 || a->mode == SR_EPI_BWD) && a->act != SR_ACT_NONE && !a->aux && a->mode == SR_EPI_BWD) return SR_EINVAL;
   if (a->mode == SR_EPI_FWD && a->naux_fwd > 0 && !a->aux) return SR_EINVAL;
   if (a->M == 0) return SR_OK;
-  if (a->M % a->group) return SR_EINVAL;
+  if (a->tangent_rows) {
+    if (a->tangent_rows != 1 || a->mode != SR_EPI_BWD || a->group != 4 || (a->act != SR_ACT_RELU && a->act != SR_ACT_NONE) || a->M % 3) return SR_EINVAL;
+  } else if (a->M % a->group) return SR_EINVAL;
   const int ncols = a->N + (a->mode == SR_EPI_FWD ? a->naux_fwd : 0);
   sr_gemm_args g = *a;
   if (g.mode != SR_EPI_FWD) g.naux_fwd = 0;
@@ -766,7 +817,7 @@
     if (a->nprob[l] < 1 || a->nprob[l] > 2) return SR_EINVAL;
     for (int p = 0; p < a->nprob[l]; ++p) {
       const sr_gemm_args& g = a->g[l][p];
-      if (!g.A || !g.B || !g.C || g.N <= 0 || g.K <= 0 || g.group != a->m_mul) return SR_EINVAL;
+      if (!g.A || !g.B || !g.C || g.N <= 0 || g.K <= 0 || g.group != a->m_mul || g.tangent_rows) return SR_EINVAL;
       if ((g.lda & 3) || (g.ldb & 3) || (g.ldc & 3) || ((uintptr_t)g.A & 15) || ((uintptr_t)g.B & 15) || ((uintptr_t)g.C & 15)) return SR_EINVAL;
       if (g.mode != SR_EPI_FWD && g.mode != SR_EPI_BWD) return SR_EINVAL;
       if (g.mode == SR_EPI_BWD && g.naux_fwd != 0) return SR_EINVAL;
@@ -797,6 +848,25 @@
   return (int64_t)splits * N * lddw;
 }
 
+static int tn_tangent_check(const sr_gemm_tn_args* a, int rows_per_split) {
+  if (!a->tangent_rows) return SR_OK;
+  if (a->tangent_rows != 1 || a->group != 4 || a->R % 3) return SR_EINVAL;
+  if (((int64_t)rows_per_split / 3 * 4 + 64) * a->lda * 4 > 0xFFFFFFFFll) return SR_EINVAL;
+  return SR_OK;
+}
+
+static int tn_rows_per_split(const sr_gemm_tn_args* a) {
+  const int64_t R = a->tangent_rows ? (int64_t)(a->R / 3) * 4 : a->R;
+  const int rows = (int)(sr_cdiv(sr_cdiv(R, a->splits), TBR) * TBR);
+  return a->tangent_rows ? rows / 4 * 3 : rows;
+}
+
+static sr_gemm_tn_args tn_kernel_args(const sr_gemm_tn_args& a) {
+  sr_gemm_tn_args g = a;
+  if (g.tangent_rows) g.db_partial = nullptr;
+  return g;
+}
+
 int sr_mlp_gemm_tn(const sr_gemm_tn_args* a, void* stream) {
   if (!a || !a->dW || !a->partial || a->R < 0 || a->N <= 0 || a->K <= 0 || a->splits < 1) return SR_EINVAL;
   if (a->R > 0 && (!a->Z || !a->A)) return SR_EINVAL;
@@ -805,21 +875,22 @@
   if ((a->db != nullptr) != (a->db_partial != nullptr) || (a->db && a->group < 1)) return SR_EINVAL;
   const bool narrow = tn_narrow(a->N, a->lddw);
   const int tiles = narrow ? (int)sr_cdiv(a->N, 256) : (int)(sr_cdiv(a->N, 128) * sr_cdiv(a->K, 128));
-  int rows_per_split = (int)sr_cdiv(a->R, a->splits);
-  rows_per_split = (int)(sr_cdiv(rows_per_split, TBR) * TBR);
+  const int rows_per_split = tn_rows_per_split(a);
+  if (tn_tangent_check(a, rows_per_split) != SR_OK) return SR_EINVAL;
+  const sr_gemm_tn_args g = tn_kernel_args(*a);
   if (a->R > 0) {
     using Narrow = TnCfg<256, 64>;
     using Square = TnCfg<128, 128>;
     if (narrow)
-      hipLaunchKernelGGL((gemm_tn_kernel<256, 64>), dim3(tiles * a->splits), dim3(256), Narrow::kLdsFloats * sizeof(float), (hipStream_t)stream, *a,
+      hipLaunchKernelGGL((gemm_tn_kernel<256, 64>), dim3(tiles * a->splits), dim3(256), Narrow::kLdsFloats * sizeof(float), (hipStream_t)stream, g,
                          rows_per_split);
     else
-      hipLaunchKernelGGL((gemm_tn_kernel<128, 128>), dim3(tiles * a->splits), dim3(256), Square::kLdsFloats * sizeof(float), (hipStream_t)stream, *a,
+      hipLaunchKernelGGL((gemm_tn_kernel<128, 128>), dim3(tiles * a->splits), dim3(256), Square::kLdsFloats * sizeof(float), (hipStream_t)stream, g,
                          rows_per_split);
   }
   const int64_t total = (int64_t)a->N * a->lddw / 4 + (a->db ? a->N : 0);
-  sr_launch_stream(slab_reduce_kernel, total, 256, stream, a->partial, a->dW, a->N, a->K, a->lddw, a->R > 0 ? a->splits : 0, a->accumulate, a->db_partial,
-                   a->db);
+  sr_launch_stream(slab_reduce_kernel, total, 256, stream, g.partial, g.dW, g.N, g.K, g.lddw, g.R > 0 ? g.splits : 0, g.accumulate, g.db_partial,
+                   g.db);
   return sr_launch_status();
 }
 
@@ -844,9 +915,9 @@
     if (rc != SR_OK) return rc;
     if (tn_narrow(p.N, p.lddw)) return SR_EINVAL;
     const int tiles = (int)(sr_cdiv(p.N, 128) * sr_cdiv(p.K, 128));
-    int rows_per_split = (int)sr_cdiv(p.R, p.splits);
-    rows_per_split = (int)(sr_cdiv(rows_per_split, TBR) * TBR);
-    G.p[i] = Rd.p[i] = p;
+    const int rows_per_split = tn_rows_per_split(&p);
+    if (tn_tangent_check(&p, rows_per_split) != SR_OK) return SR_EINVAL;
+    G.p[i] = Rd.p[i] = tn_kernel_args(p);
     G.rows_per_split[i] = Rd.rows_per_split[i] = rows_per_split;
     G.first[i] = nb; G.blocks[i] = p.R > 0 ? tiles * p.splits : 0;
     nb += (int)(sr_cdiv(G.blocks[i], 8) * 8);
diff --git a/selfreconcode_amd/mlp_engine.py b/selfreconcode_amd/mlp_engine.py
--- a/selfreconcode_amd/mlp_engine.py
+++ b/selfreconcode_amd/mlp_engine.py
@@ -12,6 +12,7 @@
 EPI_FWD, EPI_BWD = _lib.SR_EPI_FWD, _lib.SR_EPI_BWD
 
 TN_SIDE_STREAM = True
+TANGENT_SWEEP = True
 GROUP_TN_BELOW = 16384
 DEBUG_TN_DELAY_MS = int(os.environ.get("SR_DEBUG_TN_DELAY_MS", "0"))
 _TN_STREAMS = {}
@@ -149,46 +150,50 @@
 PROFILE = _GemmProfile()
 
 
-def set_gemm_args(a, A, B, C, M, N, K, bias, group, act, mode, out_scale=1.0, aux=None, naux_fwd=0, nact_bwd=0, aux_scale=1.0, pitches=None):
+def set_gemm_args(a, A, B, C, M, N, K, bias, group, act, mode, out_scale=1.0, aux=None, naux_fwd=0, nact_bwd=0, aux_scale=1.0, pitches=None,
+                  tangent_rows=0):
     lda, ldb, ldc, ldaux = pitches or (A.stride(0), B.stride(0), C.stride(0), 0 if aux is None else aux.stride(0))
     a.A, a.lda, a.B, a.ldb, a.C, a.ldc = A.data_ptr(), lda, B.data_ptr(), ldb, C.data_ptr(), ldc
     a.M, a.N, a.K = M, N, K
     a.bias = _lib.ptr(bias)
     a.group, a.act, a.mode, a.out_scale = group, act, mode, out_scale
     a.aux, a.ldaux, a.naux_fwd, a.nact_bwd, a.aux_scale = _lib.ptr(aux), ldaux, naux_fwd, nact_bwd, aux_scale
+    a.tangent_rows = tangent_rows
 
 
 def _gemm_nt(A, lda, B, ldb, C, ldc, M, N, K, bias, group, act, mode, out_scale=1.0, aux=None, ldaux=0, naux_fwd=0,
-             nact_bwd=0, aux_scale=1.0):
+             nact_bwd=0, aux_scale=1.0, tangent_rows=0):
     a = _lib.SrGemmArgs()
-    set_gemm_args(a, A, B, C, M, N, K, bias, group, act, mode, out_scale, aux, naux_fwd, nact_bwd, aux_scale, (lda, ldb, ldc, ldaux))
+    set_gemm_args(a, A, B, C, M, N, K, bias, group, act, mode, out_scale, aux, naux_fwd, nact_bwd, aux_scale, (lda, ldb, ldc, ldaux), tangent_rows)
     PROFILE.launch("sr_mlp_gemm_nt", a, _lib.stream_of(C), M >= 128 and N > 32, (M, N, K, mode, group))
 
 
-_TnProblem = collections.namedtuple("_TnProblem", "Z ldz A lda R N K lddw group dW db accumulate")
-
-
-def _tn_workspace(R, N, lddw):
+_TnProblem = collections.namedtuple("_TnProblem", "Z ldz A lda R N K lddw group dW db accumulate tangent_rows", defaults=(0,))
+
+
+def _tn_workspace(R, N, lddw, tangent_rows=0):
+    if tangent_rows:
+        R = R // 3 * 4
     splits = ctypes.c_int32(0)
     ws = _lib.raw("sr_mlp_gemm_tn_workspace_floats")(R, N, lddw, ctypes.byref(splits))
     return max(int(ws), 1), splits.value
 
 
-def _set_tn_args(a, Z, ldz, A, lda, R, N, K, lddw, group, dW, db, accumulate, partial, ws, splits):
+def _set_tn_args(a, Z, ldz, A, lda, R, N, K, lddw, group, dW, db, accumulate, tangent_rows, partial, ws, splits):
     a.Z, a.ldz, a.A, a.lda, a.dW, a.lddw, a.partial = Z.data_ptr(), ldz, A.data_ptr(), lda, dW.data_ptr(), lddw, partial
     a.R, a.N, a.K, a.splits, a.accumulate = R, N, K, splits, 1 if accumulate else 0
-    a.db, a.db_partial, a.group = db.data_ptr(), partial + 4 * ws, group
-
-
-def _gemm_tn(Z, ldz, A, lda, R, N, K, lddw, group=1, dW=None, db=None, accumulate=False):
-    ws, splits = _tn_workspace(R, N, lddw)
+    a.db, a.db_partial, a.group, a.tangent_rows = db.data_ptr(), partial + 4 * ws, group, tangent_rows
+
+
+def _gemm_tn(Z, ldz, A, lda, R, N, K, lddw, group=1, dW=None, db=None, accumulate=False, tangent_rows=0):
+    ws, splits = _tn_workspace(R, N, lddw, tangent_rows)
     if dW is None:
         dW = torch.empty((N, lddw), dtype=torch.float32, device=Z.device)
     partial = torch.empty((ws + splits * N,), dtype=torch.float32, device=Z.device)
     if db is None:
         db = torch.empty((N,), dtype=torch.float32, device=Z.device)
     a = _lib.SrGemmTnArgs()
-    _set_tn_args(a, Z, ldz, A, lda, R, N, K, lddw, group, dW, db, accumulate, partial.data_ptr(), ws, splits)
+    _set_tn_args(a, Z, ldz, A, lda, R, N, K, lddw, group, dW, db, accumulate, tangent_rows, partial.data_ptr(), ws, splits)
     PROFILE.launch("sr_mlp_gemm_tn", a, _lib.stream_of(Z), R >= 128 and N > 32, (R, N, K, "tn", group))
     return dW, db
 
@@ -203,7 +208,7 @@
     g.n = len(problems)
     sizes, total = [], 0
     for p in problems:
-        ws, splits = _tn_workspace(p.R, p.N, p.lddw)
+        ws, splits = _tn_workspace(p.R, p.N, p.lddw, p.tangent_rows)
         sizes.append((ws, splits, total))
         total += (ws + splits * p.N + 3) // 4 * 4
     partial = torch.empty((total,), dtype=torch.float32, device=problems[0].Z.device)
@@ -237,7 +242,7 @@
             _debug_delay(device, DEBUG_TN_DELAY_MS)
         if len(problems) == 1:
             p = problems[0]
-            _gemm_tn(*p[:9], dW=p.dW, db=p.db, accumulate=p.accumulate)
+            _gemm_tn(*p[:9], dW=p.dW, db=p.db, accumulate=p.accumulate, tangent_rows=p.tangent_rows)
         else:
             _gemm_tn_group(problems)
     for p in problems:
@@ -313,9 +318,25 @@
     return _DW_SINK, sink
 
 
-def reverse(spec, A0, WTs, acts, Ybar, group, need_input_grad=True, need_param_grad=True, Ws=None, bs=None):
+def tangent_sweep_applies(spec, group, need_input_grad):
+    return (TANGENT_SWEEP and group == 4 and not need_input_grad
+            and all(L.act in (ACT_RELU, ACT_NONE) and not L.nfill for L in spec.layers))
+
+
+def tangent_rows_of(Jbar):
+    P, n = Jbar.shape[0], Jbar.shape[1]
+    out = torch.zeros((3 * P, 4), dtype=torch.float32, device=Jbar.device)
+    out.view(P, 3, 4)[..., :n] = Jbar.transpose(1, 2)
+    return out
+
+
+def reverse(spec, A0, WTs, acts, Ybar, group, need_input_grad=True, need_param_grad=True, Ws=None, bs=None, tangent_only=False):
     _check_mat(Ybar, "Ybar")
     R = A0.shape[0]
+    if tangent_only and not (tangent_sweep_applies(spec, group, need_input_grad) and R % 4 == 0 and Ybar.shape[0] == R // 4 * 3):
+        raise RuntimeError(f"mlp_engine: a tangent-only sweep needs group 4, ReLU / linear layers, no input cotangent and 3 rows per sample "
+                           f"(group {group}, {Ybar.shape[0]} rows for {R})")
+    Rz, tr = Ybar.shape[0] if tangent_only else R, 1 if tangent_only else 0
     nl = len(spec.layers)
     dWs, dbs = [None] * nl, [None] * nl
     A0bar_extra = None
@@ -330,28 +351,29 @@
             if need_param_grad:
                 route, sink = _weight_gradient_route(l, L, Ws, bs, seg, grouped)
                 if sink is not None:
-                    p = _TnProblem(Zbar, Zbar.stride(0), X, X.stride(0), R, L.N, L.K, pad4(L.K), group, *sink)
+                    p = _TnProblem(Zbar, Zbar.stride(0), X, X.stride(0), Rz, L.N, L.K, pad4(L.K), group, *sink, tr)
                     if route == _DW_GROUPED:
                         grouped.append(p)
                     elif route == _DW_SIDE:
                         _launch_on_tn_stream(A0.device, [p])
                     else:
-                        _gemm_tn(*p[:9], dW=p.dW, db=p.db, accumulate=p.accumulate)
+                        _gemm_tn(*p[:9], dW=p.dW, db=p.db, accumulate=p.accumulate, tangent_rows=p.tangent_rows)
                 elif route == _DW_SEGMENTED:
                     S, rs = seg
                     dWs[0] = torch.empty((L.N, pad4(L.K)), dtype=torch.float32, device=A0.device)
                     dbs[0] = torch.zeros((S, L.N), dtype=torch.float32, device=A0.device)
+                    rz = rs // 4 * 3 if tangent_only else rs
                     for s in range(S):
-                        _gemm_tn(Zbar[s * rs:(s + 1) * rs], Zbar.stride(0), X[s * rs:(s + 1) * rs], X.stride(0), rs, L.N, L.K, pad4(L.K), group,
-                                 dW=dWs[0], db=dbs[0][s], accumulate=s > 0)
+                        _gemm_tn(Zbar[s * rz:(s + 1) * rz], Zbar.stride(0), X[s * rs:(s + 1) * rs], X.stride(0), rz, L.N, L.K, pad4(L.K), group,
+                                 dW=dWs[0], db=dbs[0][s], accumulate=s > 0, tangent_rows=tr)
                 else:
-                    dWs[l], dbs[l] = _gemm_tn(Zbar, Zbar.stride(0), X, X.stride(0), R, L.N, L.K, pad4(L.K), group)
+                    dWs[l], dbs[l] = _gemm_tn(Zbar, Zbar.stride(0), X, X.stride(0), Rz, L.N, L.K, pad4(L.K), group, tangent_rows=tr)
             if l > 0:
                 Pv = spec.layers[l - 1]
-                Znew = torch.empty((R, pad4(L.K)), dtype=torch.float32, device=A0.device)
-                _gemm_nt(Zbar, Zbar.stride(0), WTs[l], WTs[l].stride(0), Znew, Znew.stride(0), R, L.K, L.N, None, group, Pv.act,
+                Znew = torch.empty((Rz, pad4(L.K)), dtype=torch.float32, device=A0.device)
+                _gemm_nt(Zbar, Zbar.stride(0), WTs[l], WTs[l].stride(0), Znew, Znew.stride(0), Rz, L.K, L.N, None, group, Pv.act,
                          EPI_BWD, out_scale=Pv.out_scale, aux=acts[l - 1], ldaux=acts[l - 1].stride(0), nact_bwd=Pv.N,
-                         aux_scale=Pv.out_scale)
+                         aux_scale=Pv.out_scale, tangent_rows=tr)
                 if Pv.nfill and need_input_grad:
                     A0bar_extra = Znew[:, Pv.N:Pv.N + Pv.nfill]
                 Zbar = Znew
diff --git a/selfreconcode_amd/model/Deformer.py b/selfreconcode_amd/model/Deformer.py
--- a/selfreconcode_amd/model/Deformer.py
+++ b/selfreconcode_amd/model/Deformer.py
@@ -452,17 +452,21 @@
         P = flat.shape[0]
         if dbar is None and Jbar is None:
             return (None,) * (7 + 2 * nl)
-        ybar = torch.zeros((P, 4, 4), dtype=torch.float32, device=flat.device)
-        if dbar is not None:
-            ybar[:, 0, :3] = dbar.reshape(-1, 3)
-        if Jbar is not None:
-            ybar[:, 1:4, :3] = Jbar.transpose(1, 2)
         WTs = [me.transposed_of(Ws[l], spec.layers[l].K) for l in range(nl)]
         acts_full = acts + [None]
         need_par = any(ctx.needs_input_grad[7:])
         need_x = ctx.needs_input_grad[2]
         need_in = need_x or (ctx.needs_input_grad[3] and ctx.E > 0)
-        A0bar, dWs, dbs = me.reverse(spec, A0, WTs, acts_full, ybar.view(P * 4, 4), 4, need_in, need_par, Ws, list(wb[nl:]))
+        if dbar is None and me.tangent_sweep_applies(spec, 4, need_in):
+            ybar = me.tangent_rows_of(Jbar)
+            A0bar, dWs, dbs = me.reverse(spec, A0, WTs, acts_full, ybar, 4, need_in, need_par, Ws, list(wb[nl:]), tangent_only=True)
+        else:
+            ybar = torch.zeros((P, 4, 4), dtype=torch.float32, device=flat.device)
+            if dbar is not None:
+                ybar[:, 0, :3] = dbar.reshape(-1, 3)
+            if Jbar is not None:
+                ybar[:, 1:4, :3] = Jbar.transpose(1, 2)
+            A0bar, dWs, dbs = me.reverse(spec, A0, WTs, acts_full, ybar.view(P * 4, 4), 4, need_in, need_par, Ws, list(wb[nl:]))
         if not need_par:
             dWs, dbs = [None] * nl, [None] * nl
         xbar = None
```

After: 24.30, median of 6. 3.8% higher.
